# cisco/openh264

Hardware: NVIDIA B200
Metric: 1080p_encode_fps (higher is better)
Workload: dtype u8

## Files before the change

openh264_b200/csrc/enc_batch.cu:

```cuda
#include <atomic>
#include <chrono>
#include <condition_variable>
#include <functional>
#include <mutex>
#include <string.h>
#include <thread>
#include <vector>

#include "../../include/b2h264_codec.h"
#include "b2h264_internal.h"
#include "enc_host.h"
#include "enc_launch.h"
#include "host_pool.h"

using b2h264::StreamCtl;
using b2h264::Pool;
using b2h264::usable_cores;

namespace {

#define CK(x) do { cudaError_t e_ = (x); if (e_ != cudaSuccess) return (int)e_; } while (0)


}

struct b2h264_enc {
  b2h264_enc_config cfg;
  int S = 0, n_mb = 0;
  std::vector<StreamCtl> ctl;
  std::vector<uint8_t> idr_next;
  std::vector<int32_t> p_since_idr;
  std::vector<uint8_t> have_ref_p;
  int cur_rec = 0;
  std::vector<uint8_t> stream_rec;
  cudaStream_t st = nullptr;
  cudaStream_t st_in = nullptr;
  cudaStream_t st_out = nullptr;
  cudaStream_t st_dbk = nullptr;
  uint8_t* d_cur = nullptr;
  int32_t* d_vaa = nullptr;
  uint8_t* d_pic_all = nullptr;
  uint8_t* d_pic[2] = {nullptr, nullptr};
  uint8_t* d_src = nullptr;
  MbInfo* d_mbi = nullptr;
  RefMbInfo* d_rinfo[2] = {nullptr, nullptr};
  MbOut* d_out[2] = {nullptr, nullptr};
  int32_t* d_sad = nullptr;
  int32_t* d_prog = nullptr;
  int32_t* d_bits = nullptr;
  bool mb_bits_on = false;
  int* d_tickets = nullptr;
  void* d_stash = nullptr;
  StreamFrame* d_sf[2] = {nullptr, nullptr};
  alignas(64) unsigned char tmap_pic[128];
  bool have_tmap = false;
  void* d_tmap = nullptr;
  const uint8_t** d_srcptr[2] = {nullptr, nullptr};
  uint8_t* h_src = nullptr;
  MbOut* h_out[2] = {nullptr, nullptr};
  int32_t* h_idx[2] = {nullptr, nullptr};
  int32_t* h_cnt[2] = {nullptr, nullptr};
  unsigned long long last_d2h = 0;
  StreamFrame* h_sf[2] = {nullptr, nullptr};
  const uint8_t** h_srcptr[2] = {nullptr, nullptr};
  struct Slot { bool busy = false; std::vector<uint8_t> idr; std::vector<int> act;
                cudaEvent_t ev0, ev1, ev2, done, in_done, enc_done, ev_ready, ev_dbk; };
  Slot slot[2];
  int submit_idx = 0, collect_idx = 0;
  std::vector<std::vector<uint8_t>> bs;
  Pool* pool = nullptr;
  float last_us[4] = {0, 0, 0, 0};
  bool own_stream = true;
  size_t frame_bytes = 0, cur_bytes = 0, pic_bytes = 0, pic_y_bytes = 0, pic_c_bytes = 0;

  uint8_t* pic_plane0(int set, int s, int pl) const {
    const int sty = ctl[0].rec_stride_y(), stc = ctl[0].rec_stride_c();
    uint8_t* base = d_pic[set] + (size_t)s * pic_bytes;
    if (pl == 0) return base + (size_t)32 * sty + 32;
    return base + pic_y_bytes + (size_t)(pl - 1) * pic_c_bytes + (size_t)16 * stc + 16;
  }
};

extern "C" {

int b2h264_enc_create(const b2h264_enc_config* cfg, b2h264_enc** out) {
  if (!cfg || !out) return -1;
  if (cfg->width < 16 || cfg->height < 16 || (cfg->width & 3) || (cfg->height & 1) || cfg->qp < 0 || cfg->qp > 51 ||
      cfg->n_streams < 1)
    return -2;
  int rc = b2h264_init(cfg->device);
  if (rc) return rc;
  if ((rc = enc_upload_deblock_tables())) return rc;
  b2h264_enc* e = new b2h264_enc();
  e->cfg = *cfg;
  e->S = cfg->n_streams;
  e->ctl.resize(e->S);
  for (auto& c : e->ctl) {
    c.init(cfg->width, cfg->height, cfg->qp, cfg->fps, cfg->target_bitrate, cfg->entropy_cabac, cfg->profile_idc);
    c.fast_mode = cfg->complexity_low != 0;
    if (!c.set_loop_filter(cfg->loop_filter_idc, cfg->loop_filter_alpha_c0_offset, cfg->loop_filter_beta_offset)) { delete e; return -1; }
    c.increasing_ids = cfg->sps_pps_id_strategy != 0;
  }
  e->idr_next.assign(e->S, 1);
  e->p_since_idr.assign(e->S, 0);
  e->have_ref_p.assign(e->S, 0);
  e->stream_rec.assign(e->S, 0);
  const StreamCtl& c0 = e->ctl[0];
  const int mbw = c0.sp.mb_w, mbh = c0.sp.mb_h;
  e->n_mb = mbw * mbh;
  e->frame_bytes = (size_t)cfg->width * cfg->height * 3 / 2;
  e->cur_bytes = (size_t)e->n_mb * 384;
  e->pic_y_bytes = (size_t)c0.rec_stride_y() * c0.rec_rows_y();
  e->pic_c_bytes = (size_t)c0.rec_stride_c() * c0.rec_rows_c();
  e->pic_bytes = (e->pic_y_bytes + 2 * e->pic_c_bytes + 255) & ~(size_t)255;
  const size_t S = e->S;
  CK(cudaStreamCreateWithFlags(&e->st, cudaStreamNonBlocking));
  CK(cudaStreamCreateWithFlags(&e->st_in, cudaStreamNonBlocking));
  CK(cudaStreamCreateWithFlags(&e->st_dbk, cudaStreamNonBlocking));
  {
    int lo = 0, hi = 0;
    cudaDeviceGetStreamPriorityRange(&lo, &hi);
    CK(cudaStreamCreateWithPriority(&e->st_out, cudaStreamNonBlocking, lo));
  }
  CK(cudaMalloc(&e->d_pic_all, 2 * S * e->pic_bytes + 256));
  CK(cudaMemset(e->d_pic_all, 0, 2 * S * e->pic_bytes + 256));
  CK(cudaMalloc(&e->d_cur, 2 * S * e->cur_bytes + 256));
  CK(cudaMemset(e->d_cur, 0, 2 * S * e->cur_bytes + 256));
  CK(cudaMalloc(&e->d_vaa, S * e->n_mb * 4 * sizeof(int32_t)));
  CK(cudaMemset(e->d_vaa, 0, S * e->n_mb * 4 * sizeof(int32_t)));
  for (int i = 0; i < 2; i++) {
    e->d_pic[i] = e->d_pic_all + (size_t)i * S * e->pic_bytes;
    CK(cudaMalloc(&e->d_rinfo[i], S * e->n_mb * sizeof(RefMbInfo)));
    CK(cudaMemset(e->d_rinfo[i], 0, S * e->n_mb * sizeof(RefMbInfo)));
    CK(cudaMalloc(&e->d_out[i], S * e->n_mb * sizeof(MbOut)));
    CK(cudaMalloc(&e->d_sf[i], S * sizeof(StreamFrame)));
    CK(cudaMalloc(&e->d_srcptr[i], S * sizeof(uint8_t*)));
    CK(cudaHostAlloc(&e->h_out[i], S * e->n_mb * sizeof(MbOut), cudaHostAllocMapped));
    CK(cudaHostAlloc(&e->h_idx[i], S * e->n_mb * sizeof(int32_t), cudaHostAllocMapped));
    CK(cudaHostAlloc(&e->h_cnt[i], S * sizeof(int32_t), cudaHostAllocMapped));
    CK(cudaMallocHost(&e->h_sf[i], S * sizeof(StreamFrame)));
    CK(cudaMallocHost(&e->h_srcptr[i], S * sizeof(uint8_t*)));
    CK(cudaEventCreate(&e->slot[i].ev0));
    CK(cudaEventCreate(&e->slot[i].ev1));
    CK(cudaEventCreate(&e->slot[i].ev2));
    CK(cudaEventCreateWithFlags(&e->slot[i].done, cudaEventDisableTiming));
    CK(cudaEventCreateWithFlags(&e->slot[i].in_done, cudaEventDisableTiming));
    CK(cudaEventCreateWithFlags(&e->slot[i].enc_done, cudaEventDisableTiming));
    CK(cudaEventCreateWithFlags(&e->slot[i].ev_ready, cudaEventDisableTiming));
    CK(cudaEventCreateWithFlags(&e->slot[i].ev_dbk, cudaEventDisableTiming));
  }
  e->have_tmap = b2h264_make_tmap_planes(e->tmap_pic, e->d_pic_all, (uint64_t)c0.rec_stride_y(), (uint64_t)c0.rec_rows_y(), 2 * (uint64_t)S,
                                         (uint64_t)c0.rec_stride_y(), (uint64_t)e->pic_bytes, 64, 48) == 0;
  if (e->have_tmap) {
    CK(cudaMalloc(&e->d_tmap, 128));
    CK(cudaMemcpy(e->d_tmap, e->tmap_pic, 128, cudaMemcpyHostToDevice));
  }
  CK(cudaMalloc(&e->d_src, 2 * S * e->frame_bytes + 256));
  CK(cudaMallocHost(&e->h_src, 2 * S * e->frame_bytes));
  CK(cudaMalloc(&e->d_mbi, S * e->n_mb * sizeof(MbInfo)));
  CK(cudaMemset(e->d_mbi, 0, S * e->n_mb * sizeof(MbInfo)));
  CK(cudaMalloc(&e->d_sad, S * e->n_mb * sizeof(int32_t)));
  CK(cudaMemset(e->d_sad, 0, S * e->n_mb * sizeof(int32_t)));
  CK(cudaMalloc(&e->d_prog, S * 2 * mbh * sizeof(int32_t)));
  CK(cudaMalloc(&e->d_bits, S * e->n_mb * sizeof(int32_t)));
  CK(cudaMalloc(&e->d_tickets, enc_sched_ints((int)S, e->n_mb) * sizeof(int)));
  CK(cudaMalloc(&e->d_stash, enc_stash_bytes((int)S, e->ctl[0].sp.mb_h)));
  e->bs.resize(S);
  int nt = cfg->entropy_threads;
  if (nt <= 0) { nt = usable_cores(); if (nt > (int)S) nt = (int)S; if (nt < 1) nt = 1; }
  e->pool = new Pool(nt);
  *out = e;
  return 0;
}

void b2h264_enc_destroy(b2h264_enc* e) {
  if (!e) return;
  cudaSetDevice(e->cfg.device);
  cudaStreamSynchronize(e->st);
  delete e->pool;
  cudaFree(e->d_pic_all); cudaFree(e->d_cur); cudaFree(e->d_vaa); cudaFree(e->d_tmap); cudaFree(e->d_src); cudaFree(e->d_mbi); cudaFree(e->d_sad); cudaFree(e->d_prog); cudaFree(e->d_bits); cudaFree(e->d_tickets); cudaFree(e->d_stash);
  cudaFreeHost(e->h_src);
  for (int i = 0; i < 2; i++) {
    cudaFree(e->d_rinfo[i]); cudaFree(e->d_out[i]); cudaFree(e->d_sf[i]); cudaFree(e->d_srcptr[i]);
    cudaFreeHost(e->h_out[i]); cudaFreeHost(e->h_idx[i]); cudaFreeHost(e->h_cnt[i]); cudaFreeHost(e->h_sf[i]); cudaFreeHost(e->h_srcptr[i]);
    cudaEventDestroy(e->slot[i].ev0); cudaEventDestroy(e->slot[i].ev1); cudaEventDestroy(e->slot[i].ev2); cudaEventDestroy(e->slot[i].done); cudaEventDestroy(e->slot[i].in_done); cudaEventDestroy(e->slot[i].enc_done); cudaEventDestroy(e->slot[i].ev_ready); cudaEventDestroy(e->slot[i].ev_dbk);
  }
  if (e->own_stream) cudaStreamDestroy(e->st);
  cudaStreamDestroy(e->st_in); cudaStreamDestroy(e->st_out); if (e->st_dbk) cudaStreamDestroy(e->st_dbk);
  delete e;
}

int b2h264_enc_force_idr(b2h264_enc* e, int stream) {
  if (!e || stream >= e->S) return -1;
  for (int s = 0; s < e->S; s++) if (stream < 0 || stream == s) e->idr_next[s] = 1;
  return 0;
}

int b2h264_enc_submit(b2h264_enc* e, const uint8_t* const* src, int src_on_device) {
  if (!e || !src) return -1;
  CK(cudaSetDevice(e->cfg.device));
  const int k = e->submit_idx & 1;
  b2h264_enc::Slot& sl = e->slot[k];
  if (sl.busy) return -3;
  const int S = e->S, mbw = e->ctl[0].sp.mb_w, mbh = e->ctl[0].sp.mb_h;
  sl.act.clear();
  for (int s = 0; s < S; s++) if (src[s]) sl.act.push_back(s);
  const int n = (int)sl.act.size();
  if (n == 0) return -5;
  for (int i = 0; i < n; i++) {
    const int s = sl.act[i];
    if (src_on_device) { e->h_srcptr[k][i] = src[s]; continue; }
    uint8_t* dd = e->d_src + ((size_t)k * S + s) * e->frame_bytes;
    e->h_srcptr[k][i] = dd;
    cudaPointerAttributes at;
    const bool pinned = cudaPointerGetAttributes(&at, src[s]) == cudaSuccess && at.type == cudaMemoryTypeHost;
    const uint8_t* from = src[s];
    if (!pinned) {
      (void)cudaGetLastError();
      uint8_t* hs = e->h_src + ((size_t)k * S + s) * e->frame_bytes;
      memcpy(hs, src[s], e->frame_bytes);
      from = hs;
    }
    CK(cudaMemcpyAsync(dd, from, e->frame_bytes, cudaMemcpyHostToDevice, e->st_in));
  }
  sl.idr.assign(S, 0);
  for (int i = 0; i < n; i++) {
    const int s = sl.act[i];
    const bool idr = e->idr_next[s] != 0 || (e->cfg.intra_period > 0 && 1 + e->p_since_idr[s] >= e->cfg.intra_period);
    e->p_since_idr[s] = idr ? 0 : e->p_since_idr[s] + 1;
    sl.idr[s] = idr;
    StreamFrame& F = e->h_sf[k][i];
    F.p = e->ctl[s].frame_params(idr, e->have_ref_p[s] != 0);
    const int cpar = e->stream_rec[s];
    uint8_t* cur = e->d_cur + ((size_t)cpar * S + s) * e->cur_bytes;
    F.f.prev_luma = e->cfg.complexity_low ? e->d_cur + ((size_t)(1 - cpar) * S + s) * e->cur_bytes : nullptr;
    F.f.vaa_sad8x8 = e->cfg.complexity_low ? e->d_vaa + (size_t)s * e->n_mb * 4 : nullptr;
    F.f.cur[0] = cur; F.f.cur[1] = cur + (size_t)e->n_mb * 256; F.f.cur[2] = cur + (size_t)e->n_mb * 320;
    const int prec = e->stream_rec[s];
    F.p.ref_plane = (1 - prec) * S + s;
    for (int pl = 0; pl < 3; pl++) { F.f.rec[pl] = e->pic_plane0(prec, s, pl); F.f.ref[pl] = e->pic_plane0(1 - prec, s, pl); }
    F.f.mbi = e->d_mbi + (size_t)s * e->n_mb;
    F.f.rec_info = e->d_rinfo[prec] + (size_t)s * e->n_mb;
    F.f.ref_info = e->d_rinfo[1 - prec] + (size_t)s * e->n_mb;
    F.f.out = e->d_out[k] + (size_t)i * e->n_mb;
    F.f.sad_cost = e->d_sad + (size_t)s * e->n_mb;
    F.f.mb_bits = e->mb_bits_on ? e->d_bits + (size_t)s * e->n_mb : nullptr;
    e->idr_next[s] = 0;
    e->have_ref_p[s] = !idr;
  }
  for (int i = 0; i < n; i++) e->stream_rec[sl.act[i]] ^= 1;
  if (!src_on_device) {
    CK(cudaEventRecord(sl.in_done, e->st_in));
    CK(cudaStreamWaitEvent(e->st, sl.in_done, 0));
  }
  CK(cudaMemcpyAsync(e->d_sf[k], e->h_sf[k], n * sizeof(StreamFrame), cudaMemcpyHostToDevice, e->st));
  CK(cudaMemcpyAsync(e->d_srcptr[k], e->h_srcptr[k], n * sizeof(uint8_t*), cudaMemcpyHostToDevice, e->st));
  CK(cudaEventRecord(sl.ev0, e->st));
  int rc = enc_launch_frame(e->d_sf[k], e->d_srcptr[k], n, e->cfg.width, e->cfg.height, mbw, mbh, e->d_tickets, e->d_stash,
                            e->have_tmap ? e->tmap_pic : nullptr, e->d_tmap, e->cfg.complexity_low != 0, e->st, e->st_dbk, sl.ev_ready, sl.ev_dbk);
  if (rc) return rc;
  CK(cudaEventRecord(sl.ev1, e->st));
  rc = enc_launch_deblock_expand(e->d_sf[k], n, mbw, mbh, e->d_tickets, e->st, sl.ev_dbk);
  if (rc) return rc;
  CK(cudaEventRecord(sl.ev2, e->st));
  CK(cudaStreamWaitEvent(e->st_out, sl.ev1, 0));
  rc = enc_launch_pack(e->d_sf[k], n, e->n_mb, e->h_out[k], e->h_idx[k], e->h_cnt[k], e->st_out);
  if (rc) return rc;
  CK(cudaEventRecord(sl.done, e->st_out));
  sl.busy = true;
  e->submit_idx++;
  return 0;
}

int b2h264_enc_collect(b2h264_enc* e, const uint8_t** bs, int32_t* bs_bytes, int32_t* frame_type) {
  if (!e) return -1;
  CK(cudaSetDevice(e->cfg.device));
  const int k = e->collect_idx & 1;
  b2h264_enc::Slot& sl = e->slot[k];
  if (!sl.busy) return -4;
  CK(cudaEventSynchronize(sl.done));
  float ms = 0;
  cudaEventElapsedTime(&ms, sl.ev0, sl.ev1);
  e->last_us[0] = ms * 1000.f;
  if (cudaEventQuery(sl.ev2) == cudaSuccess && cudaEventElapsedTime(&ms, sl.ev1, sl.ev2) == cudaSuccess)
    e->last_us[1] = ms * 1000.f;
  (void)cudaGetLastError();
  const auto t0 = std::chrono::steady_clock::now();
  const int n_mb = e->n_mb, n = (int)sl.act.size();
  e->last_d2h = (unsigned long long)n * (n_mb + 1) * sizeof(int32_t);
  for (int i = 0; i < n; i++) e->last_d2h += (unsigned long long)e->h_cnt[k][i] * 32;
  for (int s = 0; s < e->S; s++) e->bs[s].clear();
  std::function<void(int)> job = [&](int i) {
    const int s = sl.act[i];
    e->ctl[s].write_access_unit_packed(sl.idr[s] != 0, e->h_out[k] + (size_t)i * n_mb, e->h_idx[k] + (size_t)i * n_mb, &e->bs[s]);
  };
  e->pool->run(n, job);
  e->last_us[2] = std::chrono::duration<float, std::micro>(std::chrono::steady_clock::now() - t0).count();
  std::vector<uint8_t> active(e->S, 0);
  for (int i = 0; i < n; i++) active[sl.act[i]] = 1;
  for (int s = 0; s < e->S; s++) {
    if (bs) bs[s] = active[s] ? e->bs[s].data() : nullptr;
    if (bs_bytes) bs_bytes[s] = (int32_t)e->bs[s].size();
    if (frame_type) frame_type[s] = !active[s] ? 0 : sl.idr[s] ? 1 : 2;
  }
  sl.busy = false;
  e->collect_idx++;
  return 0;
}

int b2h264_enc_reset_stream(b2h264_enc* e, int stream) {
  if (!e || stream < 0 || stream >= e->S) return -1;
  if (e->slot[0].busy || e->slot[1].busy) return -3;
  CK(cudaSetDevice(e->cfg.device));
  e->ctl[stream] = StreamCtl();
  e->ctl[stream].init(e->cfg.width, e->cfg.height, e->cfg.qp, e->cfg.fps, e->cfg.target_bitrate, e->cfg.entropy_cabac, e->cfg.profile_idc);
  e->ctl[stream].increasing_ids = e->cfg.sps_pps_id_strategy != 0;
  e->ctl[stream].fast_mode = e->cfg.complexity_low != 0;
  e->ctl[stream].set_loop_filter(e->cfg.loop_filter_idc, e->cfg.loop_filter_alpha_c0_offset, e->cfg.loop_filter_beta_offset);
  e->ctl[stream].record_mb_bits = e->mb_bits_on;
  e->idr_next[stream] = 1;
  e->p_since_idr[stream] = 0;
  e->have_ref_p[stream] = 0;
  CK(cudaMemsetAsync(e->d_sad + (size_t)stream * e->n_mb, 0, e->n_mb * sizeof(int32_t), e->st));
  for (int i = 0; i < 2; i++) CK(cudaMemsetAsync(e->d_rinfo[i] + (size_t)stream * e->n_mb, 0, e->n_mb * sizeof(RefMbInfo), e->st));
  CK(cudaMemsetAsync(e->d_mbi + (size_t)stream * e->n_mb, 0, e->n_mb * sizeof(MbInfo), e->st));
  CK(cudaStreamSynchronize(e->st));
  return 0;
}

int b2h264_enc_set_mb_bits(b2h264_enc* e, int on) {
  if (!e) return -1;
  if (e->slot[0].busy || e->slot[1].busy) return -3;
  e->mb_bits_on = on != 0;
  for (auto& c : e->ctl) c.record_mb_bits = on != 0;
  return 0;
}

int b2h264_enc_get_mb_bits(b2h264_enc* e, int stream, int32_t* device_bits, int32_t* host_bits) {
  if (!e || stream < 0 || stream >= e->S || !e->mb_bits_on) return -1;
  if (e->slot[0].busy || e->slot[1].busy) return -3;
  CK(cudaSetDevice(e->cfg.device));
  CK(cudaStreamSynchronize(e->st));
  if (device_bits) CK(cudaMemcpy(device_bits, e->d_bits + (size_t)stream * e->n_mb, e->n_mb * sizeof(int32_t), cudaMemcpyDeviceToHost));
  if (host_bits) {
    if ((int)e->ctl[stream].last_mb_bits.size() != e->n_mb) return -1;
    memcpy(host_bits, e->ctl[stream].last_mb_bits.data(), e->n_mb * sizeof(int32_t));
  }
  return 0;
}

int b2h264_enc_last_coded_mbs(b2h264_enc* e, unsigned long long* count) {
  if (!e || !count) return -1;
  unsigned long long n = 0;
  for (const auto& c : e->ctl) n += (unsigned long long)c.last_coded_mbs;
  *count = n;
  return 0;
}
int b2h264_enc_last_d2h_bytes(b2h264_enc* e, unsigned long long* bytes) {
  if (!e || !bytes) return -1;
  *bytes = e->last_d2h;
  return 0;
}

int b2h264_enc_get_recon(b2h264_enc* e, int stream, uint8_t* dst) {
  if (!e || stream < 0 || stream >= e->S || !dst) return -1;
  CK(cudaSetDevice(e->cfg.device));
  CK(cudaStreamSynchronize(e->st));
  const int set = 1 - e->stream_rec[stream];
  const int w = e->cfg.width, h = e->cfg.height;
  for (int pl = 0; pl < 3; pl++) {
    const int pw = pl ? w / 2 : w, ph = pl ? h / 2 : h;
    const int st = pl ? e->ctl[0].rec_stride_c() : e->ctl[0].rec_stride_y();
    CK(cudaMemcpy2D(dst, pw, e->pic_plane0(set, stream, pl), st, pw, ph, cudaMemcpyDeviceToHost));
    dst += (size_t)pw * ph;
  }
  return 0;
}

int b2h264_enc_last_timing(b2h264_enc* e, float* us3) {
  if (!e || !us3) return -1;
  us3[0] = e->last_us[0]; us3[1] = e->last_us[1]; us3[2] = e->last_us[2];
  return 0;
}

int b2h264_enc_set_stream(b2h264_enc* e, void* stream) {
  if (!e) return -1;
  if (e->slot[0].busy || e->slot[1].busy) return -3;
  CK(cudaStreamSynchronize(e->st));
  if (e->own_stream) cudaStreamDestroy(e->st);
  e->st = (cudaStream_t)stream;
  e->own_stream = false;
  return 0;
}

}
```

openh264_b200/csrc/enc_frame.cuh:

```cuda
#pragma once
#include "enc_mb.cuh"
#include "enc_cavlc_bits.cuh"
#ifdef B2H264_WITH_INTER
#include "enc_inter.cuh"
#endif

namespace mbk {

MBK_HD void mb_ctx(MbCtx& c, const EncFrameParams& p, const EncFramePtrs& f, int mbx, int mby) {
  static_assert(sizeof(EncFrameParams) % 4 == 0 && sizeof(EncFramePtrs) % 4 == 0, "copied as words");
  warp_sync();
  const uint32_t* sp = reinterpret_cast<const uint32_t*>(&p);
  const uint32_t* sfp = reinterpret_cast<const uint32_t*>(&f);
  uint32_t* dp = reinterpret_cast<uint32_t*>(&c.p);
  uint32_t* df = reinterpret_cast<uint32_t*>(&c.f);
  for (int i = lane_id(); i < (int)(sizeof(EncFrameParams) / 4); i += MBK_WS) dp[i] = sp[i];
  for (int i = lane_id(); i < (int)(sizeof(EncFramePtrs) / 4); i += MBK_WS) df[i] = sfp[i];
  if (lane_id() == 0) {
    c.mbx = mbx; c.mby = mby;
    c.nb = (mbx > 0 ? NB_LEFT : 0) | (mby > 0 ? NB_TOP : 0) | (mbx > 0 && mby > 0 ? NB_TOPLEFT : 0) |
           (mby > 0 && mbx < p.mb_w - 1 ? NB_TOPRIGHT : 0);
    c.qp = p.qp;
    c.qp_c = tbl_chroma_qp(p.qp);
    c.lambda = tbl_lambda(p.qp);
    c.tmap_ref = nullptr; c.wbar = nullptr; c.win_mode = 0;
  }
  warp_sync();
}

#ifndef B2H264_WITH_INTER
enum { MBS_DONE = 0, MBS_A = 1, MBS_I = 2, MBS_BSKIP = 3, MBS_B = 4, MBS_C = 5, MBS_COUNT = 6 };
#endif

MBK_HD int mb_run_stage(const MbCtx& c, MbScratch& s, int stage) {
  int next = MBS_DONE;
  if (stage == MBS_A || stage == MBS_I) {
    phase_mark(s, 31);
    uint32_t* a = reinterpret_cast<uint32_t*>(&s.info);
    for (int i = lane_id(); i < (int)(sizeof(MbInfo) / 4); i += MBK_WS) a[i] = 0;
    uint32_t* b = reinterpret_cast<uint32_t*>(&s.out);
    for (int i = lane_id(); i < MBOUT_HEADER_WORDS; i += MBK_WS) b[i] = 0;
    mb_load_all(c, s);
    phase_mark(s, 0);
  } else {
    mb_load_cur(c, s);
  }
  if (stage == MBS_I) {
    intra_mb_md_enc(c, s, 0x7fffffff);
    if (lane_id() == 0) { s.info.ref_idx = -1; c.f.sad_cost[c.mby * c.p.mb_w + c.mbx] = 0; }
  }
#ifdef B2H264_WITH_INTER
  else if (stage == MBS_A) next = inter_stage_a(c, s);
  else if (stage == MBS_B || stage == MBS_BSKIP) next = inter_stage_b(c, s);
  else if (stage == MBS_C) next = inter_stage_c(c, s);
#endif
  warp_sync();
  if (next == MBS_DONE) {
    phase_mark(s, 10);
    if (s.info.mb_type == MBT_PSKIP && s.st.is_skip != 0) mb_store_recon_skip(c, s);
    else mb_store_recon(c, s);
    mb_publish(c, s);
    if (c.f.mb_bits != nullptr) {
      const int b = mb_cavlc_bits(c, s);
      if (lane_id() == 0) c.f.mb_bits[c.mby * c.p.mb_w + c.mbx] = b;
    }
    phase_mark(s, 11);
  }
  return next;
}

MBK_HD void encode_one_mb(const EncFrameParams& p, const EncFramePtrs& f, MbScratch& s, int mbx, int mby) {
  mb_ctx(s.ctx, p, f, mbx, mby);
  int stage = p.is_idr ? MBS_I : MBS_A;
  while (stage != MBS_DONE) stage = mb_run_stage(s.ctx, s, stage);
}

}
```

openh264_b200/csrc/enc_inter.cuh:

```cuda
#pragma once
#include "enc_mb.cuh"
#include "mbk_mc.cuh"
#include "mbk_me.cuh"

namespace mbk {

#define REF_NOT_AVAIL (-2)
#define REF_NOT_IN_LIST (-1)

MBK_HD int cache30(int k) { return 7 + blk_y(k) * 6 + blk_x(k); }


MBK_HD int median3(int a, int b, int c) {
  const int mn = a < b ? a : b, mx = a < b ? b : a;
  return c < mn ? mn : (c > mx ? mx : c);
}

MBK_HD int nb_slot_bit(int k) {
  return (int)((((uint32_t)NB_TOPLEFT) | ((uint32_t)NB_TOP << 8) | ((uint32_t)NB_TOPRIGHT << 16) | ((uint32_t)NB_LEFT << 24)) >> (8 * k)) & 0xff;
}
MBK_FN void fill_inter_cache(const MbCtx& c, MbScratch& s, bool ref_ids = false) {
  for (int ci = lane_id(); ci < 30; ci += MBK_WS) {
    int k = -1, blk = 0;
    if (ci == 0) { k = 0; blk = 15; }
    else if (ci <= 4) { k = 1; blk = 12 + ci - 1; }
    else if (ci == 5) { k = 2; blk = 12; }
    else if (ci % 6 == 0) { k = 3; blk = 4 * (ci / 6 - 1) + 3; }
    int16_t mx = 0, my = 0;
    int8_t ref = 0;
    if (k >= 0) {
      const bool avail = (c.nb & nb_slot_bit(k)) != 0;
      const MbInfo* n = &s.nbi[k];
      if (avail && MBT_IS_INTER(n->mb_type)) { mx = n->mv[blk][0]; my = n->mv[blk][1]; if (ref_ids) ref = n->i4_mode[blk]; }
      else ref = avail ? REF_NOT_IN_LIST : REF_NOT_AVAIL;
    } else if (ci == 9 || ci == 11 || ci == 17 || ci == 21 || ci == 23) {
      ref = REF_NOT_AVAIL;
    }
    s.mvc[ci][0] = mx; s.mvc[ci][1] = my; s.refc[ci] = ref;
  }
  for (int k = lane_id(); k < 4; k += MBK_WS) {
    const bool avail = (c.nb & nb_slot_bit(k)) != 0;
    const MbInfo* n = &s.nbi[k];
    const bool inter = avail && MBT_IS_INTER(n->mb_type);
    const bool skip = inter && n->mb_type == MBT_PSKIP;
    s.sadc[k] = inter ? s.nb_sad[k] : 0;
    s.skip_flag[k] = skip;
    s.sad_skip[k] = skip ? s.nb_skip_sad[k] : 0;
  }
  warp_sync();
}

MBK_FN void pred_mv(const MbScratch& s, int blk , int part_w, int ref, int* px, int* py) {
  const int left = cache30(blk) - 1, top = cache30(blk) - 6;
  const int lr = s.refc[left], tr = s.refc[top], rtr = s.refc[top + part_w];
  int dr, dmx, dmy;
  if (rtr == REF_NOT_AVAIL) { dr = s.refc[top - 1]; dmx = s.mvc[top - 1][0]; dmy = s.mvc[top - 1][1]; }
  else { dr = rtr; dmx = s.mvc[top + part_w][0]; dmy = s.mvc[top + part_w][1]; }
  if (tr == REF_NOT_AVAIL && dr == REF_NOT_AVAIL && lr != REF_NOT_AVAIL) { *px = s.mvc[left][0]; *py = s.mvc[left][1]; return; }
  const int match = (ref == lr ? 1 : 0) | (ref == tr ? 2 : 0) | (ref == dr ? 4 : 0);
  if (match == 1) { *px = s.mvc[left][0]; *py = s.mvc[left][1]; }
  else if (match == 2) { *px = s.mvc[top][0]; *py = s.mvc[top][1]; }
  else if (match == 4) { *px = dmx; *py = dmy; }
  else { *px = median3(s.mvc[left][0], s.mvc[top][0], dmx); *py = median3(s.mvc[left][1], s.mvc[top][1], dmy); }
}
MBK_HD void pred_16x8_mv(const MbScratch& s, int blk, int ref, int* px, int* py) {
  if (blk == 0) { if (ref == s.refc[1]) { *px = s.mvc[1][0]; *py = s.mvc[1][1]; return; } }
  else { if (ref == s.refc[18]) { *px = s.mvc[18][0]; *py = s.mvc[18][1]; return; } }
  pred_mv(s, blk, 4, ref, px, py);
}
MBK_HD void pred_8x16_mv(const MbScratch& s, int blk, int ref, int* px, int* py) {
  if (blk == 0) { if (ref == s.refc[6]) { *px = s.mvc[6][0]; *py = s.mvc[6][1]; return; } }
  else {
    int di = 5;
    if (s.refc[5] == REF_NOT_AVAIL) di = 2;
    if (ref == s.refc[di]) { *px = s.mvc[di][0]; *py = s.mvc[di][1]; return; }
  }
  pred_mv(s, blk, 2, ref, px, py);
}
MBK_HD void pred_skip_mv(const MbScratch& s, int* px, int* py, int ref0 = 0 ) {
  const int lr = s.refc[6], tr = s.refc[1];
  if (lr == REF_NOT_AVAIL || tr == REF_NOT_AVAIL || (lr == ref0 && s.mvc[6][0] == 0 && s.mvc[6][1] == 0) ||
      (tr == ref0 && s.mvc[1][0] == 0 && s.mvc[1][1] == 0)) { *px = 0; *py = 0; return; }
  pred_mv(s, 0, 4, ref0, px, py);
}
MBK_HD void cache_set(MbScratch& s, int blk, int w4, int h4, int mvx, int mvy, int ref = 0) {
  if (lane_id() == 0) {
    const int c0 = cache30(blk);
    for (int y = 0; y < h4; y++)
      for (int x = 0; x < w4; x++) { s.mvc[c0 + 6 * y + x][0] = (int16_t)mvx; s.mvc[c0 + 6 * y + x][1] = (int16_t)mvy; s.refc[c0 + 6 * y + x] = (int8_t)ref; }
  }
  warp_sync();
}
MBK_HD void mb_mv_set(MbScratch& s, int blk, int w4, int h4, int mvx, int mvy) {
  if (lane_id() == 0) {
    const int x0 = blk_x(blk), y0 = blk_y(blk);
    for (int y = 0; y < h4; y++)
      for (int x = 0; x < w4; x++) { s.info.mv[(y0 + y) * 4 + x0 + x][0] = (int16_t)mvx; s.info.mv[(y0 + y) * 4 + x0 + x][1] = (int16_t)mvy; }
  }
  warp_sync();
}

MBK_HD int predict_sad(const MbScratch& s) {
  const int rb = s.refc[1], ra = s.refc[6];
  int rc = s.refc[5], sc = s.sadc[2];
  const int sb = s.sadc[1], sa = s.sadc[3];
  if (rc == REF_NOT_AVAIL) { rc = s.refc[0]; sc = s.sadc[0]; }
  int pred;
  if (rb == REF_NOT_AVAIL && rc == REF_NOT_AVAIL && ra != REF_NOT_AVAIL) pred = sa;
  else {
    const int m = (0 == ra ? 1 : 0) | (0 == rb ? 2 : 0) | (0 == rc ? 4 : 0);
    pred = m == 1 ? sa : m == 2 ? sb : m == 4 ? sc : median3(sa, sb, sc);
  }
  const int t = pred << 6;
  return ((t - (t >> 3) + (t >> 5)) + 32) >> 6;
}
MBK_HD int predict_sad_skip(const MbScratch& s) {
  const int rb = s.refc[1], ra = s.refc[6];
  int rc = s.refc[5];
  const int sb = s.skip_flag[1] ? s.sad_skip[1] : 0, sa = s.skip_flag[3] ? s.sad_skip[3] : 0;
  int sc = s.skip_flag[2] ? s.sad_skip[2] : 0, rskip = s.skip_flag[2];
  if (rc == REF_NOT_AVAIL) { rc = s.refc[0]; sc = s.skip_flag[0] ? s.sad_skip[0] : 0; rskip = s.skip_flag[0]; }
  if (rb == REF_NOT_AVAIL && rc == REF_NOT_AVAIL && ra != REF_NOT_AVAIL) return sa;
  const int m = ((0 == ra && s.skip_flag[3]) ? 1 : 0) | ((0 == rb && s.skip_flag[1]) ? 2 : 0) | ((0 == rc && rskip) ? 4 : 0);
  return m == 1 ? sa : m == 2 ? sb : m == 4 ? sc : median3(sa, sb, sc);
}

MBK_HD const uint8_t* ref_luma(const MbCtx& c, int px, int py) {
  return c.f.ref[0] + (ptrdiff_t)(c.mby * 16 + py) * c.p.rec_stride_y + c.mbx * 16 + px;
}
MBK_HD const uint8_t* ref_chroma(const MbCtx& c, int pl, int px, int py) {
  return c.f.ref[pl] + (ptrdiff_t)(c.mby * 8 + py) * c.p.rec_stride_c + c.mbx * 8 + px;
}

MBK_STAGE void mc_chroma_part(const MbCtx& c, uint8_t* dst , int ox, int oy, int w, int h, int mvx, int mvy) {
  const int cx = ox >> 1, cy = oy >> 1;
  MBK_NO_UNROLL
  for (int pl = 0; pl < 2; pl++) {
    const uint8_t* src = ref_chroma(c, 1 + pl, cx + (mvx >> 3), cy + (mvy >> 3));
    warp_mc_chroma(src, c.p.rec_stride_c, dst + 64 * pl + cy * 8 + cx, 8, mvx, mvy, w >> 1, h >> 1);
  }
  warp_sync();
}

struct SkipResult { bool ok; int cost_luma; int cost_skip; int mvx, mvy; };

MBK_STAGE bool try_py_skip(const MbCtx& c, MbScratch& s) {
  const int16_t* ff = tbl_quant_ff(c.qp);
  const int16_t* mf = tbl_quant_mf(c.qp);
  int big = 0, ctr = 0;
  for (int k = lane_id(); k < 16; k += MBK_WS) {
    int16_t d[16], l[16];
    for (int i = 0; i < 16; i++) d[i] = s.coef[16 * k + i];
    const uint16_t mx = (uint16_t)quant4x4_max(d, ff, mf);
    if (mx > 1) big = 1;
    else if (mx == 1) { scan4x4_dcac(l, d); ctr += single_ctr4x4(l); }
  }
  big = warp_sum(big); ctr = warp_sum(ctr);
  return big == 0 && ctr < 6;
}
MBK_STAGE bool try_puv_skip(const MbCtx& c, MbScratch& s, int uv) {
  const int16_t* res = s.coef + 256 + 64 * uv;
  const int16_t* ff = tbl_quant_ff(c.qp_c);
  const int16_t* mf = tbl_quant_mf(c.qp_c);
  const int16_t dcin[4] = {res[0], res[16], res[32], res[48]};
  const bool dc_fail = hadamard_quant2x2_skip(dcin, (int16_t)(ff[0] << 1), (int16_t)(mf[0] >> 1)) != 0;
  int big = 0, ctr = 0;
  for (int j = lane_id(); j < 4; j += MBK_WS) {
    int16_t d[16], l[16];
    for (int i = 0; i < 16; i++) d[i] = res[16 * j + i];
    const uint16_t mx = (uint16_t)quant4x4_max(d, ff, mf);
    if (mx > 1) big = 1;
    else if (mx == 1) { scan4x4_ac(l, d); ctr += single_ctr4x4(l); }
  }
  big = warp_sum(big); ctr = warp_sum(ctr);
  return !dc_fail && big == 0 && ctr < 7;
}
MBK_FN void dct_luma_mb(MbScratch& s, const uint8_t* pred ) {
  for (int k = lane_id(); k < 16; k += MBK_WS) {
    int16_t d[16];
    const int o = blk_y(k) * 4 * 16 + blk_x(k) * 4;
    dct4x4(d, s.cur_y + o, 16, pred + o, 16);
    for (int i = 0; i < 16; i++) s.coef[16 * k + i] = d[i];
  }
  warp_sync();
}

MBK_STAGE SkipResult pskip_enc(const MbCtx& c, MbScratch& s, int sad_pred_skip, int ref_mb_type) {
  SkipResult r;
  r.ok = false; r.cost_luma = 0; r.cost_skip = 0;
  int mvx, mvy;
  pred_skip_mv(s, &mvx, &mvy);
  r.mvx = mvx; r.mvy = mvy;
  const int ix = mvx >> 2, iy = mvy >> 2;
  int n = c.mbx * 16 + ix;
  if (n < -29 || n > c.p.mb_w * 16 + 12) return r;
  n = c.mby * 16 + iy;
  if (n < -29 || n > c.p.mb_h * 16 + 12) return r;
  uint8_t* py = s.skip_pred;
  phase_mark(s, 12);
  warp_mc_luma(ref_luma(c, ix, iy), c.p.rec_stride_y, py, 16, mvx, mvy, 16, 16);
  warp_sync();
  phase_mark(s, 13);
  const int sad_y = warp_sad(s.cur_y, 16, py, 16, 4, 4);
  MBK_NO_UNROLL
  for (int pl = 0; pl < 2; pl++)
    warp_mc_chroma(ref_chroma(c, 1 + pl, ix >> 1, iy >> 1), c.p.rec_stride_c, s.skip_pred + 256 + 64 * pl, 8, mvx, mvy, 8, 8);
  warp_sync();
  const int sad_c = warp_sad(s.cur_c, 8, s.skip_pred + 256, 8, 3, 3) + warp_sad(s.cur_c + 64, 8, s.skip_pred + 320, 8, 3, 3);
  const int sad_mb = sad_y + sad_c;
  phase_mark(s, 14);
  bool ok = sad_mb == 0 || sad_mb < sad_pred_skip ||
            (c.p.ref_is_p && ref_mb_type == MBT_PSKIP && sad_mb < c.f.ref_info[c.mby * c.p.mb_w + c.mbx].skip_sad);
  if (!ok) {
    dct_luma_mb(s, py);
    if (try_py_skip(c, s)) {
      for (int t = lane_id(); t < 4; t += MBK_WS) {
        int16_t d[16];
        const int ox = (t & 1) * 4, oy = (t >> 1) * 4;
        dct4x4(d, s.cur_c + oy * 8 + ox, 8, s.skip_pred + 256 + oy * 8 + ox, 8);
        for (int i = 0; i < 16; i++) s.coef[256 + 16 * t + i] = d[i];
      }
      warp_sync();
      bool uv_ok = true;
      MBK_NO_UNROLL
      for (int uv = 0; uv < 2 && uv_ok; uv++) {
        if (uv) {
          for (int t = lane_id(); t < 4; t += MBK_WS) {
            int16_t d[16];
            const int ox = (t & 1) * 4, oy = (t >> 1) * 4;
            dct4x4(d, s.cur_c + 64 + oy * 8 + ox, 8, s.skip_pred + 320 + oy * 8 + ox, 8);
            for (int i = 0; i < 16; i++) s.coef[320 + 16 * t + i] = d[i];
          }
          warp_sync();
        }
        uv_ok = try_puv_skip(c, s, uv);
      }
      ok = uv_ok;
    }
  }
  phase_mark(s, 15);
  if (ok) {
    r.ok = true;
    if (c.p.fast_mode) {
      r.cost_luma = sad_y;
      if (lane_id() == 0) c.f.sad_cost[c.mby * c.p.mb_w + c.mbx] = sad_y;
    } else {
      r.cost_luma = warp_satd_inl(s.cur_y, 16, py, 16, 4, 4);
    }
    phase_mark(s, 16);
    r.cost_skip = sad_mb;
  }
  return r;
}

MBK_HD void win_issue(const MbCtx& c, MbScratch& s, int sx, int sy) {
#ifdef __CUDA_ARCH__
  warp_sync();
  if (c.win_mode == 0) { if (lane_id() == 0) s.win_ok = 0; warp_sync(); return; }
  const int X = (32 + c.mbx * 16 + sx - 16) & ~15, Y = 32 + c.mby * 16 + sy - 16, Z = c.p.ref_plane;
  const int wx0 = X - 32 - c.mbx * 16;
  if (lane_id() == 0) { s.win_x0 = wx0; s.win_y0 = sy - 16; s.win_ok = 1; }
  if (c.win_mode == 1) {
    if (lane_id() == 0) {
      const uint32_t dst = (uint32_t)__cvta_generic_to_shared(scratch_win(s));
      const uint32_t bar = (uint32_t)__cvta_generic_to_shared(&c.wbar->bar);
      asm volatile("fence.proxy.async.shared::cta;" ::: "memory");
      asm volatile("{ .reg .b64 st; mbarrier.arrive.expect_tx.shared::cta.b64 st, [%0], %1; }" ::"r"(bar), "r"(WIN_W * WIN_H) : "memory");
      asm volatile("cp.async.bulk.tensor.3d.shared::cluster.global.mbarrier::complete_tx::bytes [%0], [%1, {%2, %3, %4}], [%5];"
                   ::"r"(dst), "l"(c.tmap_ref), "r"(X), "r"(Y), "r"(Z), "r"(bar) : "memory");
    }
  } else {
    const uint32_t* src = reinterpret_cast<const uint32_t*>(ref_luma(c, wx0, sy - 16));
    uint32_t* dst = reinterpret_cast<uint32_t*>(scratch_win(s));
    const int rs4 = c.p.rec_stride_y >> 2;
#pragma unroll 8
    for (int i = lane_id(); i < WIN_H * (WIN_W / 4); i += MBK_WS) {
      const int r = i / (WIN_W / 4), w = i - r * (WIN_W / 4);
      dst[i] = src[(ptrdiff_t)r * rs4 + w];
    }
  }
  warp_sync();
#else
  (void)c; (void)sx; (void)sy;
  s.win_ok = 0;
#endif
}
MBK_HD void win_wait(const MbCtx& c, MbScratch& s) {
#ifdef __CUDA_ARCH__
  if (c.win_mode == 1 && s.win_ok) {
    const uint32_t bar = (uint32_t)__cvta_generic_to_shared(&c.wbar->bar);
    const uint32_t ph = c.wbar->phase;
    uint32_t ok = 0;
    while (!ok)
      asm volatile("{ .reg .pred p; mbarrier.try_wait.parity.shared::cta.b64 p, [%1], %2; selp.u32 %0, 1, 0, p; }"
                   : "=r"(ok) : "r"(bar), "r"(ph) : "memory");
    warp_sync();
    if (lane_id() == 0) c.wbar->phase = ph ^ 1;
    warp_sync();
  }
#else
  (void)c; (void)s;
#endif
}

MBK_STAGE void me_partition(const MbCtx& c, MbScratch& s, int blk_size, int ox, int oy, int mvp_x, int mvp_y, uint32_t sad_pred,
                         int n_mvc, const int16_t* mvc, MeState* st) {
  MeIn in;
  in.enc = s.cur_y + oy * 16 + ox; in.enc_stride = 16;
  in.ref = ref_luma(c, ox, oy); in.ref_stride = c.p.rec_stride_y;
  in.blk = blk_size;
  in.mvp_x = mvp_x; in.mvp_y = mvp_y;
  const int r = c.p.mv_range;
  const int lo_x = -((c.mbx + 1) << 4) + 3, lo_y = -((c.mby + 1) << 4) + 3;
  const int hi_x = ((c.p.mb_w - c.mbx) << 4) - 3, hi_y = ((c.p.mb_h - c.mby) << 4) - 3;
  in.min_x = lo_x > -r ? lo_x : -r; in.min_y = lo_y > -r ? lo_y : -r;
  in.max_x = hi_x < r ? hi_x : r; in.max_y = hi_y < r ? hi_y : r;
  in.n_mvc = n_mvc; in.mvc = mvc;
  in.sad_pred = sad_pred;
  in.lambda = c.lambda;
  in.calc_satd = !c.p.fast_mode;
  in.win = s.win_ok ? scratch_win(s) : nullptr;
  in.win_w = WIN_W; in.win_h = WIN_H;
  in.win_dx = s.win_x0 - ox; in.win_dy = s.win_y0 - oy;
  MeOut o;
  warp_me_search(in, o);
  if (lane_id() == 0) {
    st->mv_x = o.mv_x; st->mv_y = o.mv_y; st->mvp_x = mvp_x; st->mvp_y = mvp_y;
    st->sad_cost = o.sad_cost; st->satd_cost = o.satd_cost;
    st->satd = (int)o.satd_cost - mvd_cost(c.lambda, o.mv_x - mvp_x, o.mv_y - mvp_y);
    st->ref = o.ref_best;
  }
  warp_sync();
}
MBK_HD void me_start_point(const MbCtx& c, int mvp_x, int mvp_y, int* sx, int* sy) {
  const int r = c.p.mv_range;
  const int lo_x = -((c.mbx + 1) << 4) + 3, lo_y = -((c.mby + 1) << 4) + 3;
  const int hi_x = ((c.p.mb_w - c.mbx) << 4) - 3, hi_y = ((c.p.mb_h - c.mby) << 4) - 3;
  *sx = clip3((2 + mvp_x) >> 2, lo_x > -r ? lo_x : -r, hi_x < r ? hi_x : r);
  *sy = clip3((2 + mvp_y) >> 2, lo_y > -r ? lo_y : -r, hi_y < r ? hi_y : r);
}

struct QpelPlanes { const uint8_t* g; const uint8_t* hh; const uint8_t* vv; const uint8_t* cc; };
enum { QP_STRIDE = 32 };
MBK_HD void qpel_pair(const QpelPlanes& q, int dx, int dy, const uint8_t** pa, const uint8_t** pb) {
  const int ix = dx < 0 ? -1 : 0, iy = dy < 0 ? -1 : 0, fx = dx & 3, fy = dy & 3;
  const uint8_t* G = q.g + (iy + 3) * QP_STRIDE + (ix + 3);
  const uint8_t* H = q.hh + (iy + 1) * QP_STRIDE + (ix + 1);
  const uint8_t* V = q.vv + (iy + 1) * QP_STRIDE + (ix + 1);
  const uint8_t* C = q.cc + (iy + 1) * QP_STRIDE + (ix + 1);
  const int x3 = fx == 3 ? 1 : 0, y3 = fy == 3 ? QP_STRIDE : 0;
  if ((fx | fy) == 0) { *pa = G; *pb = G; }
  else if (fy == 0) { *pa = H; *pb = fx == 2 ? H : G + x3; }
  else if (fx == 0) { *pa = V; *pb = fy == 2 ? V : G + y3; }
  else if (fx == 2 && fy == 2) { *pa = C; *pb = C; }
  else if (fx == 2) { *pa = H + y3; *pb = C; }
  else if (fy == 2) { *pa = V + x3; *pb = C; }
  else { *pa = H + y3; *pb = V + x3; }
}

MBK_STAGE void me_refine(const MbCtx& c, MbScratch& s, MeState* st, int ox, int oy, int w, int h, uint8_t* dst) {
  const int lw = w == 16 ? 4 : 3, lh = h == 16 ? 4 : 3;
  const uint8_t* enc = s.cur_y + oy * 16 + ox;
  const int rs = c.p.rec_stride_y;
  const int px = st->mvp_x, py = st->mvp_y;
  const int mv0x = st->mv_x, mv0y = st->mv_y;
  const uint8_t* ref0 = st->ref;
  int best = (c.p.fast_mode ? warp_satd(enc, 16, ref0, rs, lw, lh) : st->satd) + mvd_cost(c.lambda, mv0x - px, mv0y - py);
  uint8_t* win = reinterpret_cast<uint8_t*>(s.coef);
  static_assert(sizeof(s.coef) >= 22 * QP_STRIDE, "window aliases the coefficient buffer");
  const int ww = w + 6, wh = h + 6, wq = (ww + 3) >> 2;
  const uint8_t* src = ref0 - (ptrdiff_t)3 * rs - 3;
  int srs = rs;
  if (s.win_ok) {
    const int x0 = ox + (mv0x >> 2) - 3 - s.win_x0, y0 = oy + (mv0y >> 2) - 3 - s.win_y0;
    if (x0 >= 0 && y0 >= 0 && x0 + 4 * wq <= WIN_W && y0 + wh <= WIN_H) { src = scratch_win(s) + y0 * WIN_W + x0; srs = WIN_W; }
  }
#ifdef __CUDA_ARCH__
  {
    uint32_t v[5];
#pragma unroll
    for (int k = 0; k < 5; k++) {
      const int i = lane_id() + 32 * k;
      const int r = i / wq, q4 = (i - r * wq) << 2;
      v[k] = i < wq * wh ? ld4u(src + (ptrdiff_t)r * srs + q4) : 0u;
    }
    warp_sync();
#pragma unroll
    for (int k = 0; k < 5; k++) {
      const int i = lane_id() + 32 * k;
      if (i < wq * wh) {
        const int r = i / wq, q4 = (i - r * wq) << 2;
        uint8_t* d = win + r * QP_STRIDE + q4;
        d[0] = (uint8_t)v[k]; d[1] = (uint8_t)(v[k] >> 8); d[2] = (uint8_t)(v[k] >> 16); d[3] = (uint8_t)(v[k] >> 24);
      }
    }
  }
#else
  for (int i = lane_id(); i < wq * wh; i += MBK_WS) {
    const int r = i / wq, q4 = (i - r * wq) << 2;
    const uint32_t v = ld4u(src + (ptrdiff_t)r * srs + q4);
    uint8_t* d = win + r * QP_STRIDE + q4;
    d[0] = (uint8_t)v; d[1] = (uint8_t)(v >> 8); d[2] = (uint8_t)(v >> 16); d[3] = (uint8_t)(v >> 24);
  }
#endif
  warp_sync();
  if (lane_id() == 0) s.win_ok = 0;
  warp_sync();
  uint8_t* ph = s.qplane[0];
  uint8_t* pv = s.qplane[1];
  uint8_t* pc = s.qplane[2];
  for (int i = lane_id(); i < (w + 1) * (h + 2); i += MBK_WS) {
    const int r = i / (w + 1), x = i - r * (w + 1);
    ph[r * QP_STRIDE + x] = (uint8_t)half_h(win + (r + 2) * QP_STRIDE + (x + 2));
  }
  for (int i = lane_id(); i < (w + 2) * (h + 1); i += MBK_WS) {
    const int r = i / (w + 2), x = i - r * (w + 2);
    pv[r * QP_STRIDE + x] = (uint8_t)half_v(win + (r + 2) * QP_STRIDE + (x + 2), QP_STRIDE);
  }
  warp_sync();
  QpelPlanes q;
  q.g = win; q.hh = ph; q.vv = pv; q.cc = pc;
  auto eval = [&](int dx, int dy) {
    const uint8_t *a, *b;
    qpel_pair(q, dx, dy, &a, &b);
    return warp_satd_avg(enc, 16, a, b, QP_STRIDE, lw, lh) + mvd_cost(c.lambda, mv0x + dx - px, mv0y + dy - py);
  };
  int hx = 0, hy = 0;
  {
    int bi = -1;
    MBK_NO_UNROLL
    for (int i = 0; i < 4; i++) {
      const int cst = eval(i == 2 ? -2 : i == 3 ? 2 : 0, i == 0 ? -2 : i == 1 ? 2 : 0);
      if (cst < best) { best = cst; bi = i; }
    }
    if (bi >= 0) { hx = bi == 2 ? -2 : bi == 3 ? 2 : 0; hy = bi == 0 ? -2 : bi == 1 ? 2 : 0; }
  }
  if (hx | hy) {
    for (int i = lane_id(); i < (w + 1) * (h + 1); i += MBK_WS) {
      const int r = i / (w + 1), x = i - r * (w + 1);
      pc[r * QP_STRIDE + x] = (uint8_t)half_c(win + (r + 2) * QP_STRIDE + (x + 2), QP_STRIDE);
    }
    warp_sync();
  }
  int fx = hx, fy = hy;
  {
    int bi = -1;
    MBK_NO_UNROLL
    for (int i = 0; i < 4; i++) {
      const int cst = eval(hx + (i == 2 ? -1 : i == 3 ? 1 : 0), hy + (i == 0 ? -1 : i == 1 ? 1 : 0));
      if (cst < best) { best = cst; bi = i; }
    }
    if (bi >= 0) { fx += (bi == 2 ? -1 : bi == 3 ? 1 : 0); fy += (bi == 0 ? -1 : bi == 1 ? 1 : 0); }
  }
  {
    const uint8_t *a, *b;
    qpel_pair(q, fx, fy, &a, &b);
    const int gsh = lw - 2;
    for (int g = lane_id(); g < (w * h) >> 2; g += MBK_WS) {
      const int y = g >> gsh, x = (g & ((1 << gsh) - 1)) << 2;
      const uint32_t v = vavgu4(ld4u(a + y * QP_STRIDE + x), ld4u(b + y * QP_STRIDE + x));
      uint8_t* d = dst + y * 16 + x;
      d[0] = (uint8_t)v; d[1] = (uint8_t)(v >> 8); d[2] = (uint8_t)(v >> 16); d[3] = (uint8_t)(v >> 24);
    }
    warp_sync();
  }
  if (lane_id() == 0) { st->mv_x = mv0x + fx; st->mv_y = mv0y + fy; st->satd_cost = (uint32_t)best; }
  warp_sync();
}

MBK_STAGE void enc_inter_y(const MbCtx& c, MbScratch& s) {
  const int16_t* ff = tbl_quant_ff(c.qp);
  const int16_t* mf = tbl_quant_mf(c.qp);
  for (int k = lane_id(); k < 16; k += MBK_WS) {
    int16_t d[16], l[16];
    for (int i = 0; i < 16; i++) d[i] = s.coef[16 * k + i];
    const int16_t mx = quant4x4_max(d, ff, mf);
    if (mx == 0) { for (int i = 0; i < 16; i++) l[i] = 0; }
    else scan4x4_dcac(l, d);
    for (int i = 0; i < 16; i++) { s.coef[16 * k + i] = d[i]; s.out.luma[k][i] = l[i]; }
    s.red[k] = mx;
    s.red[16 + k] = mx == 0 ? 0 : single_ctr4x4(l);
  }
  warp_sync();
  int ctr8[4], ctr_mb = 0;
  for (int i = 0; i < 4; i++) {
    ctr8[i] = 0;
    for (int j = 0; j < 4; j++) {
      const int mx = s.red[4 * i + j];
      if (mx == 0) continue;
      if (mx > 1) ctr8[i] += 9;
      else if (ctr8[i] < 6) ctr8[i] += s.red[16 + 4 * i + j];
    }
    ctr_mb += ctr8[i];
  }
  for (int i = lane_id(); i < 16; i += MBK_WS) s.info.nnz[i] = 0;
  warp_sync();
  if (ctr_mb < 6) {
    for (int i = lane_id(); i < 256; i += MBK_WS) s.coef[i] = 0;
  } else {
    for (int k = lane_id(); k < 16; k += MBK_WS) {
      if (ctr8[k >> 2] >= 4) {
        s.info.nnz[blk_raster(k)] = (int8_t)nonzero_count(s.out.luma[k]);
        int16_t d[16];
        for (int i = 0; i < 16; i++) d[i] = s.coef[16 * k + i];
        dequant4x4(d, tbl_dequant(c.qp));
        for (int i = 0; i < 16; i++) s.coef[16 * k + i] = d[i];
      } else {
        for (int i = 0; i < 16; i++) s.coef[16 * k + i] = 0;
      }
    }
    if (lane_id() == 0)
      for (int i = 0; i < 4; i++) if (ctr8[i] >= 4) s.info.cbp |= (uint8_t)(1 << i);
  }
  warp_sync();
}

MBK_FN void rec_luma_inter(MbScratch& s, const uint8_t* pred) {
  for (int k = lane_id(); k < 16; k += MBK_WS) {
    int16_t d[16];
    for (int i = 0; i < 16; i++) d[i] = s.coef[16 * k + i];
    const int oy = blk_y(k) * 4, ox = blk_x(k) * 4;
    idct4x4_rec(tile_y(s.tile, ox, oy), TY_PITCH, pred + oy * 16 + ox, 16, d);
  }
  warp_sync();
}

MBK_HD void decided_pskip(const MbCtx& c, MbScratch& s) {
  (void)c;
  if (lane_id() == 0) {
    s.info.mb_type = MBT_PSKIP;
    s.info.cbp = 0;
  }
  for (int i = lane_id(); i < 24; i += MBK_WS) s.info.nnz[i] = 0;
  warp_sync();
}

enum { MBS_DONE = 0, MBS_A = 1, MBS_I = 2, MBS_BSKIP = 3, MBS_B = 4, MBS_C = 5, MBS_COUNT = 6 };

MBK_FN void inter_tail(const MbCtx& c, MbScratch& s) {
  const int idx = c.mby * c.p.mb_w + c.mbx;
  const int final_type = s.st.final_type, p16_mvx = s.st.p16_mvx, p16_mvy = s.st.p16_mvy, cost_skip_mb = s.st.cost_skip_mb;
  if (lane_id() == 0) {
    s.info.mb_type = (uint8_t)final_type;
    s.info.p16x16_mv[0] = (int16_t)p16_mvx; s.info.p16x16_mv[1] = (int16_t)p16_mvy;
    if (MBT_IS_INTER(final_type)) s.info.ref_idx = 0;
    RefMbInfo ri;
    ri.mv16[0] = (int16_t)p16_mvx; ri.mv16[1] = (int16_t)p16_mvy;
    ri.skip_sad = final_type == MBT_PSKIP ? cost_skip_mb : 0;
    ri.mb_type = (uint8_t)final_type;
    ri.pad[0] = ri.pad[1] = ri.pad[2] = 0;
    c.f.rec_info[idx] = ri;
  }
  warp_sync();
}

MBK_HD void st_save(MbScratch& s, int is_skip, int cost_luma, int cost_skip_mb, int p16_mvx, int p16_mvy, int final_type) {
  warp_sync();
  if (lane_id() == 0) {
    s.st.is_skip = is_skip; s.st.cost_luma = cost_luma; s.st.cost_skip_mb = cost_skip_mb;
    s.st.p16_mvx = p16_mvx; s.st.p16_mvy = p16_mvy; s.st.final_type = final_type;
  }
  warp_sync();
}

MBK_STAGE int inter_stage_a(const MbCtx& c, MbScratch& s) {
  const int mbw = c.p.mb_w, idx = c.mby * mbw + c.mbx;
  fill_inter_cache(c, s);
  mbk_batch_sync(5, c.batch_n);
  phase_mark(s, 1);
  const int ref_mb_type = c.p.ref_is_p ? c.f.ref_info[idx].mb_type : 0xff;
  int p16_mvx = 0, p16_mvy = 0;
  const bool sk_l = (c.nb & NB_LEFT) && s.nbi[3].mb_type == MBT_PSKIP;
  const bool sk_t = (c.nb & NB_TOP) && s.nbi[1].mb_type == MBT_PSKIP;
  const bool sk_tl = (c.nb & NB_TOPLEFT) && s.nbi[0].mb_type == MBT_PSKIP;
  const bool sk_tr = (c.nb & NB_TOPRIGHT) && s.nbi[2].mb_type == MBT_PSKIP;
  const bool try_skip = sk_l || sk_t || sk_tl || sk_tr;
  const bool keep_skip = sk_l && sk_t && sk_tr;
  int cost_luma = 0, cost_skip_mb = 0;
  bool is_skip = false;
  if ((c.p.ref_is_p && ref_mb_type == MBT_PSKIP) || try_skip) {
    const SkipResult r = pskip_enc(c, s, predict_sad_skip(s), ref_mb_type);
    if (r.ok) {
      is_skip = true;
      cost_luma = r.cost_luma; cost_skip_mb = r.cost_skip;
      p16_mvx = r.mvx; p16_mvy = r.mvy;
      mb_mv_set(s, 0, 4, 4, r.mvx, r.mvy);
    }
  }
  mbk_batch_sync(6, c.batch_n);
  phase_mark(s, 2);
  if (is_skip && keep_skip) {
    decided_pskip(c, s);
    st_save(s, 1, cost_luma, cost_skip_mb, p16_mvx, p16_mvy, MBT_PSKIP);
    inter_tail(c, s);
    return MBS_DONE;
  }
  st_save(s, is_skip ? 1 : 0, cost_luma, cost_skip_mb, p16_mvx, p16_mvy, MBT_P16x16);
  return is_skip ? MBS_BSKIP : MBS_B;
}

MBK_STAGE int inter_stage_b(const MbCtx& c, MbScratch& s) {
  const int mbw = c.p.mb_w, idx = c.mby * mbw + c.mbx;
  const bool is_skip = s.st.is_skip != 0;
  int cost_luma = s.st.cost_luma, cost_skip_mb = s.st.cost_skip_mb, p16_mvx = s.st.p16_mvx, p16_mvy = s.st.p16_mvy;
  MeState& me16 = s.me[0];
  MeState* me16x8 = &s.me[1];
  MeState* me8x16 = &s.me[3];
  MeState* me8x8 = &s.me[5];
  int final_type = MBT_P16x16;
  int sad_pred_mb = 0;
  if (lane_id() == 0) s.win_ok = 0;
  warp_sync();
  int16_t (*mvc)[2] = s.mvcand;
  int px16 = 0, py16 = 0, n16 = 1;
  if (!is_skip) {
    pred_mv(s, 0, 4, 0, &px16, &py16);
    {
      int sx, sy;
      me_start_point(c, px16, py16, &sx, &sy);
      win_issue(c, s, sx, sy);
    }
    sad_pred_mb = predict_sad(s);
    n16 += (c.nb & NB_LEFT) ? 1 : 0;
    n16 += (c.nb & NB_TOP) ? 1 : 0;
    if (c.p.ref_is_p) { n16 += c.mbx < mbw - 1 ? 1 : 0; n16 += c.mby < c.p.mb_h - 1 ? 1 : 0; }
    if (lane_id() == 0) {
      int k = 0;
      mvc[k][0] = 0; mvc[k][1] = 0; k++;
      if (c.nb & NB_LEFT) { mvc[k][0] = s.nbi[3].p16x16_mv[0]; mvc[k][1] = s.nbi[3].p16x16_mv[1]; k++; }
      if (c.nb & NB_TOP) { mvc[k][0] = s.nbi[1].p16x16_mv[0]; mvc[k][1] = s.nbi[1].p16x16_mv[1]; k++; }
      if (c.p.ref_is_p) {
        if (c.mbx < mbw - 1) { mvc[k][0] = c.f.ref_info[idx + 1].mv16[0]; mvc[k][1] = c.f.ref_info[idx + 1].mv16[1]; k++; }
        if (c.mby < c.p.mb_h - 1) { mvc[k][0] = c.f.ref_info[idx + mbw].mv16[0]; mvc[k][1] = c.f.ref_info[idx + mbw].mv16[1]; k++; }
      }
    }
    warp_sync();
    win_wait(c, s);
  }
  int plan[3] = {0, 0, 0}, n_plan = 0, cost = 0;
  int rounds_run = 0;
  MBK_NO_UNROLL
  for (int t = -1; t < n_plan; t++) {
    const int shape = t < 0 ? 0 : plan[t];
    int cst = 0;
    if (t >= 0 || !is_skip) {
      const int np = shape == 0 ? 1 : shape == 3 ? 4 : 2;
      MeState* arr = shape == 0 ? &me16 : shape == 1 ? me16x8 : shape == 2 ? me8x16 : me8x8;
      MBK_NO_UNROLL
      for (int i = 0; i < np; i++) {
        int px = px16, py = py16, ox = 0, oy = 0, blk = BLK_16x16, ci = 0, cw = 4, ch = 4, ncand = n16;
        uint32_t sp = (uint32_t)sad_pred_mb;
        if (shape == 1) { pred_16x8_mv(s, 8 * i, 0, &px, &py); oy = 8 * i; blk = BLK_16x8; ci = 8 * i; ch = 2; sp = (uint32_t)(sad_pred_mb >> 1); ncand = 1; }
        else if (shape == 2) { pred_8x16_mv(s, 4 * i, 0, &px, &py); ox = 8 * i; blk = BLK_8x16; ci = 4 * i; cw = 2; sp = (uint32_t)(sad_pred_mb >> 1); ncand = 1; }
        else if (shape == 3) { pred_mv(s, 4 * i, 2, 0, &px, &py); ox = (i & 1) * 8; oy = (i >> 1) * 8; blk = BLK_8x8; ci = 4 * i; cw = 2; ch = 2; sp = (uint32_t)(sad_pred_mb >> 2); ncand = 1; }
        me_partition(c, s, blk, ox, oy, px, py, sp, ncand, &mvc[0][0], &arr[i]);
        if (shape != 0) cache_set(s, ci, cw, ch, arr[i].mv_x, arr[i].mv_y);
        cst += (int)arr[i].satd_cost;
      }
    }
    if (t >= 0) {
      mbk_batch_sync(7 + t, c.batch_n_fine);
      rounds_run = t + 1;
      if (t == 0) { if (cst < cost_luma) { cost = cst; final_type = shape == 3 ? MBT_P8x8 : shape == 1 ? MBT_P16x8 : MBT_P8x16; } else break; }
      else if (cst <= cost) { cost = cst; final_type = shape == 1 ? MBT_P16x8 : MBT_P8x16; }
      continue;
    }
    if (!is_skip) { p16_mvx = me16.mv_x; p16_mvy = me16.mv_y; cost_luma = cst; }
    if (!is_skip) mbk_batch_sync(2, c.batch_n);
    phase_mark(s, 3);
    {
      int bb;
      const int cost16 = md_i16x16_inl(c, s, &bb);
      phase_mark(s, 4);
      if (cost16 < cost_luma) {
        st_save(s, is_skip ? 1 : 0, cost_luma, cost_skip_mb, p16_mvx, p16_mvy, final_type);
        if (lane_id() == 0) { s.st.cost16 = cost16; s.st.bb = bb; }
        warp_sync();
        if (!is_skip) {
          mbk_batch_leave(3, c.batch_n); mbk_batch_leave(4, c.batch_n);
          for (int r = 0; r < 3; r++) mbk_batch_leave(7 + r, c.batch_n_fine);
        }
        return MBS_C;
      }
    }
    if (is_skip) {
      decided_pskip(c, s);
      st_save(s, 1, cost_luma, cost_skip_mb, p16_mvx, p16_mvy, MBT_PSKIP);
      inter_tail(c, s);
      return MBS_DONE;
    }
    int vaa_sign = 0;
    if (c.p.fast_mode) {
      const int32_t* v = c.f.vaa_sad8x8 + 4 * idx;
      const int b0 = v[0], b1 = v[1], b2 = v[2], b3 = v[3], avg = (b0 + b1 + b2 + b3) >> 2;
      const int d0 = (b0 >> 6) - (avg >> 6), d1 = (b1 >> 6) - (avg >> 6), d2 = (b2 >> 6) - (avg >> 6), d3 = (b3 >> 6) - (avg >> 6);
      if (d0 * d0 + d1 * d1 + d2 * d2 + d3 * d3 < 20) vaa_sign = 15;
      else vaa_sign = (b0 > avg ? 8 : 0) | (b1 > avg ? 4 : 0) | (b2 > avg ? 2 : 0) | (b3 > avg ? 1 : 0);
    }
    if (c.p.fast_mode && vaa_sign == 15) n_plan = 0;
    else if (c.p.fast_mode && (vaa_sign == 3 || vaa_sign == 12)) { plan[0] = 1; n_plan = 1; }
    else if (c.p.fast_mode && (vaa_sign == 5 || vaa_sign == 10)) { plan[0] = 2; n_plan = 1; }
    else if (c.p.fast_mode && (vaa_sign == 6 || vaa_sign == 9)) { plan[0] = 3; n_plan = 1; }
    else { plan[0] = 3; plan[1] = 1; plan[2] = 2; n_plan = 3; }
  }
  {
    for (int r = rounds_run; r < 3; r++) mbk_batch_leave(7 + r, c.batch_n_fine);
    mbk_batch_sync(3, c.batch_n);
    phase_mark(s, 6);
    uint8_t* pl = s.pred_y[0];
    uint8_t* pc = s.pred_c[0];
    int best_sad = 0;
    {
      const int shape = final_type == MBT_P16x16 ? 0 : final_type == MBT_P16x8 ? 1 : final_type == MBT_P8x16 ? 2 : 3;
      const int np = shape == 0 ? 1 : shape == 3 ? 4 : 2;
      MeState* arr = shape == 0 ? &me16 : shape == 1 ? me16x8 : shape == 2 ? me8x16 : me8x8;
      if (shape == 3) {
        if (lane_id() == 0) { s.refc[9] = s.refc[21] = REF_NOT_AVAIL; }
        warp_sync();
      }
      MBK_NO_UNROLL
      for (int i = 0; i < np; i++) {
        int ox = 0, oy = 0, w = 16, h = 16, ci = 0, cw = 4, ch = 4;
        if (shape != 0) {
          int qx, qy;
          if (shape == 1) { pred_16x8_mv(s, 8 * i, 0, &qx, &qy); oy = 8 * i; h = 8; ci = 8 * i; ch = 2; }
          else if (shape == 2) { pred_8x16_mv(s, 4 * i, 0, &qx, &qy); ox = 8 * i; w = 8; ci = 4 * i; cw = 2; }
          else { pred_mv(s, 4 * i, 2, 0, &qx, &qy); ox = (i & 1) * 8; oy = (i >> 1) * 8; w = 8; h = 8; ci = 4 * i; cw = 2; ch = 2; }
          if (lane_id() == 0) { arr[i].mvp_x = qx; arr[i].mvp_y = qy; }
          warp_sync();
        }
        me_refine(c, s, &arr[i], ox, oy, w, h, pl + oy * 16 + ox);
        cache_set(s, ci, cw, ch, arr[i].mv_x, arr[i].mv_y);
        mb_mv_set(s, ci, cw, ch, arr[i].mv_x, arr[i].mv_y);
        if (lane_id() == 0) { s.out.mvd[i][0] = (int16_t)(arr[i].mv_x - arr[i].mvp_x); s.out.mvd[i][1] = (int16_t)(arr[i].mv_y - arr[i].mvp_y); }
        best_sad += (int)arr[i].sad_cost;
        mc_chroma_part(c, pc, ox, oy, w, h, arr[i].mv_x, arr[i].mv_y);
      }
      if (shape == 0)
        cost_skip_mb = warp_sad(s.cur_y, 16, pl, 16, 4, 4) + warp_sad(s.cur_c, 8, pc, 8, 3, 3) + warp_sad(s.cur_c + 64, 8, pc + 64, 8, 3, 3);
    }
    if (lane_id() == 0) c.f.sad_cost[idx] = best_sad;
    mbk_batch_sync(4, c.batch_n);
    phase_mark(s, 7);
    if (lane_id() == 0) s.info.cbp = 0;
    warp_sync();
    dct_luma_mb(s, pl);
    enc_inter_y(c, s);
    dct_chroma(s, pc);
    enc_rec_uv(c, s, 0, true);
    enc_rec_uv(c, s, 1, true);
    rec_luma_inter(s, pl);
    rec_chroma(s, pc);
    if (final_type == MBT_P16x16 && s.info.cbp == 0) {
      int sx, sy;
      pred_skip_mv(s, &sx, &sy);
      if (sx == me16.mv_x && sy == me16.mv_y) final_type = MBT_PSKIP;
    }
    if (lane_id() == 0) s.info.mb_type = (uint8_t)final_type;
    warp_sync();
  }
  phase_mark(s, 8);
  st_save(s, 0, cost_luma, cost_skip_mb, p16_mvx, p16_mvy, final_type);
  inter_tail(c, s);
  return MBS_DONE;
}

MBK_STAGE int inter_stage_c(const MbCtx& c, MbScratch& s) {
  const int idx = c.mby * c.p.mb_w + c.mbx;
  const int bb = s.st.bb;
  int cost = s.st.cost16;
  {
    {
      bool use_i4 = false;
      if (lane_id() == 0) { s.info.mb_type = MBT_I16x16; s.info.cbp = 0; }
      warp_sync();
      fill_i4_cache(c, s);
      if (intra_try_i4x4(c, s)) {
        const int cost4 = md_enc_i4x4(c, s, cost);
        if (cost4 < cost) { use_i4 = true; cost = cost4; if (lane_id() == 0) s.info.mb_type = MBT_I4x4; warp_sync(); }
      }
      if (!use_i4) {
    if (lane_id() == 0) s.info.cbp = 0;
    warp_sync();
    enc_rec_i16x16(c, s, s.pred_y[bb]);
  }
      int cb;
      md_chroma(c, s, &cb);
      dct_chroma(s, s.pred_c[cb]);
      enc_rec_uv(c, s, 0, false);
      enc_rec_uv(c, s, 1, false);
      rec_chroma(s, s.pred_c[cb]);
      if (lane_id() == 0) { c.f.sad_cost[idx] = 0; s.info.ref_idx = REF_NOT_IN_LIST; }
      phase_mark(s, 5);
    }
  }
  warp_sync();
  if (lane_id() == 0) s.st.final_type = s.info.mb_type;
  warp_sync();
  inter_tail(c, s);
  return MBS_DONE;
}

MBK_FN void inter_mb_md_enc(const MbCtx& c, MbScratch& s) {
  int nx = inter_stage_a(c, s);
  if (nx == MBS_B || nx == MBS_BSKIP) nx = inter_stage_b(c, s);
  if (nx == MBS_C) inter_stage_c(c, s);
}

}
```

openh264_b200/csrc/enc_kernels.cu:

```cuda
#include <cuda.h>
#include <type_traits>
#include <stddef.h>
#include <stdlib.h>
#include <string.h>

#include "b2h264_internal.h"
#define B2H264_WITH_INTER 1
#include "enc_deblock.cuh"
#include "enc_frame.cuh"
#include "dec_mb.cuh"
#include "enc_launch.h"

using namespace mbk;

namespace mbk {
__constant__ uint8_t c_alpha[52];
__constant__ uint8_t c_beta[52];
__constant__ uint8_t c_tc0[52][3];
}

#define DEC_WPC 24
#ifndef ENC_WPC
#define ENC_WPC 23
#endif

__device__ __forceinline__ int ld_volatile(const int* p) { return *reinterpret_cast<const volatile int*>(p); }

__global__ void k_pad_source(const StreamFrame* __restrict__ sf, const uint8_t* const* __restrict__ src, int w, int h) {
  const StreamFrame& F = sf[blockIdx.z];
  const uint8_t* yuv = src[blockIdx.z];
  const int W = F.p.mb_w * 16, H = F.p.mb_h * 16;
  const int x = (blockIdx.x * blockDim.x + threadIdx.x) * 4, y = blockIdx.y * blockDim.y + threadIdx.y;
  if (x >= W || y >= H) return;
  uchar4 v = make_uchar4(0, 0, 0, 0);
  if (y < h) {
    const uint8_t* r = yuv + (size_t)y * w;
    if (x + 3 < w) v = *reinterpret_cast<const uchar4*>(r + x);
  }
  *reinterpret_cast<uchar4*>(const_cast<uint8_t*>(F.f.cur[0]) + (size_t)y * F.p.cur_stride_y + x) = v;
  if (y < H / 2 && x < W / 2) {
    const int cw = w / 2, ch = h / 2;
    for (int pl = 0; pl < 2; pl++) {
      uchar4 c = make_uchar4(0x80, 0x80, 0x80, 0x80);
      const uint8_t* p = yuv + (size_t)w * h + (size_t)pl * cw * ch + (size_t)y * cw;
      if (y < ch) {
        uint8_t t[4];
        for (int i = 0; i < 4; i++) t[i] = (x + i < cw) ? p[x + i] : 0x80;
        c = make_uchar4(t[0], t[1], t[2], t[3]);
      }
      *reinterpret_cast<uchar4*>(const_cast<uint8_t*>(F.f.cur[1 + pl]) + (size_t)y * F.p.cur_stride_c + x) = c;
    }
  }
}

__global__ void __launch_bounds__(256) k_vaa_sad8x8(const StreamFrame* __restrict__ sf, int n_mb) {
  const int lane = threadIdx.x & 31, mb = blockIdx.x * (blockDim.x >> 5) + (threadIdx.x >> 5);
  if (mb >= n_mb) return;
  const StreamFrame& F = sf[blockIdx.y];
  if (F.f.vaa_sad8x8 == nullptr || F.f.prev_luma == nullptr) return;
  const int st = F.p.cur_stride_y, mbx = mb % F.p.mb_w, mby = mb / F.p.mb_w;
  const size_t off = (size_t)(mby * 16 + (lane >> 1)) * st + mbx * 16 + (lane & 1) * 8;
  const uint2 a = *reinterpret_cast<const uint2*>(F.f.cur[0] + off), b = *reinterpret_cast<const uint2*>(F.f.prev_luma + off);
  int v = (int)(__vsadu4(a.x, b.x) + __vsadu4(a.y, b.y));
  v += __shfl_xor_sync(0xffffffffu, v, 2);
  v += __shfl_xor_sync(0xffffffffu, v, 4);
  v += __shfl_xor_sync(0xffffffffu, v, 8);
  if ((lane & 14) == 0) const_cast<int32_t*>(F.f.vaa_sad8x8)[(size_t)mb * 4 + (lane >> 4) * 2 + (lane & 1)] = v;
}

struct Sched {
  int* dep;
  int* queue;
  int* head;
  int* tail;
};

__device__ __forceinline__ void sched_push(const Sched& q, int id) {
  const int slot = atomicAdd(q.tail, 1);
  *reinterpret_cast<volatile int*>(q.queue + slot) = id;
}
__device__ __forceinline__ void sched_notify(const Sched& q, int id, int need) {
  if (atomicAdd(q.dep + id, 1) + 1 == need) sched_push(q, id);
}

template <class Body>
__device__ __forceinline__ void run_mbs(const StreamFrame* sf, int n_streams, const Sched q, Body body) {
  const int lane = threadIdx.x & 31;
  const int mb_w = sf[0].p.mb_w, mb_h = sf[0].p.mb_h, n_mb = mb_w * mb_h, total = n_streams * n_mb;
  for (;;) {
    int id = 0;
    if (lane == 0) {
      const int t = atomicAdd(q.head, 1);
      id = -1;
      if (t < total) {
        while ((id = ld_volatile(q.queue + t)) < 0) __nanosleep(100);
      }
    }
    id = __shfl_sync(MBK_FULL, id, 0);
    if (id < 0) break;
    __threadfence();
    const int si = id / n_mb, mb = id - si * n_mb, y = mb / mb_w, x = mb - y * mb_w;
    body(sf[si], x, y);
    __threadfence();
    __syncwarp();
    if (lane == 0) {
      if (x + 1 < mb_w) sched_notify(q, id + 1, 1 + (y > 0));
      if (y + 1 < mb_h) {
        if (x > 0) sched_notify(q, id + mb_w - 1, 1 + (x - 1 > 0));
        if (x == mb_w - 1) sched_notify(q, id + mb_w, 1 + (x > 0));
      }
    }
  }
}

enum { NQ = MBS_COUNT - 1 };
struct EncSched {
  int* dep;
  int* queue;
  int* ctl;
  uint4* stash;
  int* rowprog;
};
__device__ __forceinline__ int* ctl_head(const EncSched& q, int k) { return q.ctl + 32 * k; }
__device__ __forceinline__ int* ctl_tail(const EncSched& q, int k) { return q.ctl + 32 * k + 1; }
__device__ __forceinline__ int* ctl_done(const EncSched& q) { return q.ctl + 32 * NQ; }
constexpr int kCtlInts = 32 * (NQ + 1);
constexpr int kStashU4 = kParkSlot / 16, kCoreU4 = kParkCore / 16;
static_assert(kParkSlot % 16 == 0 && kParkCore % 16 == 0, "parked ranges are copied as uint4");
__device__ __forceinline__ void park_extra(int stage, int* off, int* n) {
  if (stage == MBS_BSKIP) { *off = (int)(offsetof(MbScratch, skip_pred) / 16); *n = 384 / 16; }
  else if (stage == MBS_C) { *off = (int)(offsetof(MbScratch, pred_y) / 16); *n = 512 / 16; }
  else { *off = 0; *n = 0; }
}

__device__ __forceinline__ void esched_push(const EncSched& q, int total, int stage, int id) {
  const int k = stage - 1;
  const int slot = atomicAdd(ctl_tail(q, k), 1);
  *reinterpret_cast<volatile int*>(q.queue + (size_t)k * total + slot) = id;
}

__device__ unsigned long long g_batch_stats[NQ + 1][3];
__device__ unsigned long long g_task_wall[NQ][2];
__device__ unsigned long long g_fill_stats[NQ][ENC_WPC + 1][2];
extern "C" int b2h264_debug_task_wall(unsigned long long* out, int reset) {
  cudaError_t e = cudaMemcpyFromSymbol(out, g_task_wall, sizeof(g_task_wall));
  if (e == cudaSuccess && reset) { unsigned long long z[NQ][2] = {}; e = cudaMemcpyToSymbol(g_task_wall, z, sizeof(z)); }
  return (int)e;
}
extern "C" int b2h264_debug_fill_stats(unsigned long long* out, int* n_lists, int* wpc, int reset) {
  *n_lists = NQ; *wpc = ENC_WPC;
  cudaError_t e = cudaMemcpyFromSymbol(out, g_fill_stats, sizeof(g_fill_stats));
  if (reset) { void* a = nullptr; if (cudaGetSymbolAddress(&a, g_fill_stats) == cudaSuccess) cudaMemset(a, 0, sizeof(g_fill_stats)); }
  return (int)e;
}
extern "C" int b2h264_debug_batch_stats(unsigned long long* out, int reset) {
  cudaError_t e = cudaMemcpyFromSymbol(out, g_batch_stats, sizeof(g_batch_stats));
  if (e == cudaSuccess && reset) { unsigned long long z[NQ + 1][3] = {}; e = cudaMemcpyToSymbol(g_batch_stats, z, sizeof(z)); }
  return (int)e;
}

template <class Body>
__device__ __forceinline__ void run_task(const StreamFrame* sf, const EncSched& q, MbScratch& s, int id, int stage, int mb_w, int mb_h,
                                         int total, int batch_n, Body& body) {
  const int lane = threadIdx.x & 31, n_mb = mb_w * mb_h;
  __threadfence();
  const int si = id / n_mb, mb = id - si * n_mb, y = mb / mb_w, x = mb - y * mb_w;
  uint4* park = q.stash + (size_t)(si * mb_h + y) * kStashU4;
  uint4* sc = reinterpret_cast<uint4*>(&s);
  if (stage != MBS_A && stage != MBS_I) {
    int xo, xn;
    park_extra(stage, &xo, &xn);
    for (int i = lane; i < kCoreU4 + xn; i += 32) {
      const uint4 v = __ldcg(park + i);
      if (i < kCoreU4) sc[i] = v; else sc[xo + i - kCoreU4] = v;
    }
    __syncwarp();
  }
  const int next = body(sf[si], x, y, stage, batch_n);
  __syncwarp();
  if (next == MBS_DONE) {
    __threadfence();
    if (lane == 0) {
      const int first = sf[si].p.is_idr ? MBS_I : MBS_A;
      const bool nr = x + 1 < mb_w;
      const bool nbl = y + 1 < mb_h && x > 0;
      const bool nb = y + 1 < mb_h && x == mb_w - 1;
      const int r0 = nr ? atomicAdd(q.dep + id + 1, 1) : 0;
      const int r1 = nbl ? atomicAdd(q.dep + id + mb_w - 1, 1) : 0;
      const int r2 = nb ? atomicAdd(q.dep + id + mb_w, 1) : 0;
      if (nr && r0 + 1 == 1 + (y > 0)) esched_push(q, total, first, id + 1);
      if (nbl && r1 + 1 == 1 + (x - 1 > 0)) esched_push(q, total, first, id + mb_w - 1);
      if (nb && r2 + 1 == 1 + (x > 0)) esched_push(q, total, first, id + mb_w);
      if (q.rowprog) atomicAdd(q.rowprog + si * mb_h + y, 1);
      atomicAdd(ctl_done(q), 1);
    }
  } else {
    int xo, xn;
    park_extra(next, &xo, &xn);
    for (int i = lane; i < kCoreU4 + xn; i += 32) park[i] = i < kCoreU4 ? sc[i] : sc[xo + i - kCoreU4];
    __threadfence();
    __syncwarp();
    if (lane == 0) esched_push(q, total, next, id);
  }
}

struct BatchSlot { int k, base, n, pad; };
constexpr int kEncThreads = 32 * (ENC_WPC + 1);
__device__ __forceinline__ void enc_cta_barrier() { asm volatile("barrier.sync 1, %0;" ::"n"(kEncThreads) : "memory"); }

template <class Body>
__device__ __forceinline__ void run_stages(const StreamFrame* sf, int n_streams, const EncSched q, MbScratch& s, int stats, bool legacy_claim, Body body) {
  __shared__ BatchSlot s_slot[2];
  __shared__ int s_ids[2][ENC_WPC];
  __shared__ int s_fin[2];
  const int lane = threadIdx.x & 31, warp = threadIdx.x >> 5;
  const int mb_w = sf[0].p.mb_w, mb_h = sf[0].p.mb_h, n_mb = mb_w * mb_h, total = n_streams * n_mb;
  if (warp == ENC_WPC) {
    int p = 0, run_n = 0;
    for (;;) {
      if (lane == 0) {
        int k = 0, h = 0, n = 0;
        long long t_exposed = 0;
        bool exposed = false;
        unsigned long long n_poll = 0, n_fail = 0, n_idle = 0;
        for (;;) {
          const int fin = run_n ? *reinterpret_cast<volatile int*>(&s_fin[p ^ 1]) : 0;
          const bool all_done = fin >= run_n;
          if (stats && all_done && !exposed) { exposed = true; t_exposed = clock64(); }
          n_poll++;
          int c[2 * NQ + 1];
#pragma unroll
          for (int kk = 0; kk < NQ; kk++)
            asm volatile("ld.volatile.global.v2.s32 {%0, %1}, [%2];" : "=r"(c[kk]), "=r"(c[NQ + kk]) : "l"(ctl_head(q, kk)) : "memory");
          asm volatile("ld.volatile.global.s32 %0, [%1];" : "=r"(c[2 * NQ]) : "l"(ctl_done(q)) : "memory");
          if (c[2 * NQ] >= total) { n = -1; break; }
          int best = -1, best_avail = 0;
#pragma unroll
          for (int kk = NQ - 1; kk >= 0; kk--) {
            const int avail = c[NQ + kk] - c[kk];
            if (avail >= ENC_WPC && best_avail < ENC_WPC) { best = kk; best_avail = avail; }
            else if (best_avail < ENC_WPC && avail > best_avail) { best = kk; best_avail = avail; }
          }
          const bool full = best_avail >= ENC_WPC;
          const bool take = best >= 0 && (all_done || (!legacy_claim && full && (fin > 0 || best_avail >= 2 * ENC_WPC)));
          if (take) {
            int tail = 0;
#pragma unroll
            for (int kk = 0; kk < NQ; kk++) if (kk == best) { h = c[kk]; tail = c[NQ + kk]; }
            bool got = false;
            for (;;) {
              n = min(ENC_WPC, tail - h);
              if (n <= 0 || (n < ENC_WPC && !all_done)) break;
              const int old = atomicCAS(ctl_head(q, best), h, h + n);
              if (old == h) { got = true; break; }
              n_fail++;
              h = old;
            }
            if (got) { k = best; break; }
            __nanosleep(100 + 40 * (blockIdx.x & 7));
            continue;
          }
          n_idle++;
          __nanosleep(all_done ? 100 : fin > 0 ? 400 : 1500);
        }
        s_slot[p].k = k; s_slot[p].base = h; s_slot[p].n = n;
        s_fin[p] = 0;
        if (stats) {
          if (exposed) atomicAdd(&g_batch_stats[NQ][2], (unsigned long long)(clock64() - t_exposed));
          atomicAdd(&g_batch_stats[NQ][0], n_poll + (n_fail << 32));
          atomicAdd(&g_batch_stats[NQ][1], n_idle);
        }
      }
      __syncwarp();
      {
        const int kk = s_slot[p].k, nn = s_slot[p].n;
        if (lane < nn) {
          int id;
          while ((id = ld_volatile(q.queue + (size_t)kk * total + s_slot[p].base + lane)) < 0) {}
          s_ids[p][lane] = id;
        }
      }
      __syncwarp();
      enc_cta_barrier();
      run_n = s_slot[p].n;
      if (run_n < 0) break;
      p ^= 1;
    }
    return;
  }
  int p = 0, prev_k = -1, prev_n = 0;
  long long t_prev = 0;
  for (;;) {
    enc_cta_barrier();
    const int k = s_slot[p].k, n = s_slot[p].n;
    if (stats && threadIdx.x == 0) {
      const long long t = clock64();
      if (prev_k >= 0) {
        const unsigned long long dt = (unsigned long long)(t - t_prev);
        atomicAdd(&g_batch_stats[prev_k][0], 1ull);
        atomicAdd(&g_batch_stats[prev_k][1], (unsigned long long)prev_n);
        atomicAdd(&g_batch_stats[prev_k][2], dt);
        atomicAdd(&g_fill_stats[prev_k][min(prev_n, ENC_WPC)][0], 1ull);
        atomicAdd(&g_fill_stats[prev_k][min(prev_n, ENC_WPC)][1], dt);
      }
      t_prev = t; prev_k = k; prev_n = n;
    }
    if (n < 0) break;
    if (warp < n) {
      const long long t_task = stats ? clock64() : 0;
      const int id = s_ids[p][warp];
      run_task(sf, q, s, id, k + 1, mb_w, mb_h, total, n, body);
      if (lane == 0) atomicAdd(&s_fin[p], 1);
      if (stats && lane == 0) { atomicAdd(&g_task_wall[k][0], (unsigned long long)(clock64() - t_task)); atomicAdd(&g_task_wall[k][1], 1ull); }
    }
    p ^= 1;
  }
}

__global__ void k_esched_init(EncSched q, const StreamFrame* __restrict__ sf, int n_streams, int n_mb) {
  const int i = blockIdx.x * blockDim.x + threadIdx.x;
  if (i == 0) {
    int na = 0, ni = 0;
    const int total = n_streams * n_mb;
    for (int s = 0; s < n_streams; s++) {
      if (sf[s].p.is_idr) q.queue[(size_t)(MBS_I - 1) * total + ni++] = s * n_mb;
      else q.queue[(size_t)(MBS_A - 1) * total + na++] = s * n_mb;
    }
    for (int k = 0; k < kCtlInts; k++) q.ctl[k] = 0;
    *ctl_tail(q, MBS_A - 1) = na;
    *ctl_tail(q, MBS_I - 1) = ni;
  }
}

__global__ void k_sched_init(Sched q, int n_streams, int n_mb) {
  const int i = blockIdx.x * blockDim.x + threadIdx.x;
  if (i < n_streams) q.queue[i] = i * n_mb;
  if (i == 0) { *q.head = 0; *q.tail = n_streams; }
}

__device__ unsigned long long g_enc_stats[16];
#ifdef B2H264_PHASE_STATS
namespace mbk { __device__ unsigned long long g_phase[32]; }
extern "C" int b2h264_debug_phase_stats(unsigned long long* out32, int reset) {
  cudaError_t e = cudaMemcpyFromSymbol(out32, mbk::g_phase, sizeof(mbk::g_phase));
  if (e == cudaSuccess && reset) { unsigned long long z[32] = {0}; e = cudaMemcpyToSymbol(mbk::g_phase, z, sizeof(z)); }
  return (int)e;
}
#endif

#ifndef ENC_MIN_CTAS
#define ENC_MIN_CTAS 1
#endif
constexpr size_t kScratchSmem = sizeof(MbScratch) * DEC_WPC + 128;
static_assert(DEC_WPC >= ENC_WPC, "one scratch area size for both kernels");
__device__ __forceinline__ MbScratch& my_scratch(uint8_t* smem) {
  const uintptr_t a = (reinterpret_cast<uintptr_t>(smem) + 127) & ~uintptr_t(127);
  return reinterpret_cast<MbScratch*>(a)[threadIdx.x >> 5];
}

__global__ void __launch_bounds__(kEncThreads, ENC_MIN_CTAS) k_encode_mbs(const StreamFrame* __restrict__ sf, int n_streams, EncSched q, int stats,
                                                                          const __grid_constant__ CUtensorMap tm_ref, const void* tm_global,
                                                                          int win_mode ,
                                                                          int* started ) {
  extern __shared__ __align__(128) uint8_t smem[];
  if (threadIdx.x == 0 && started) *reinterpret_cast<volatile int*>(started) = 1;
  __shared__ WinBar s_wbar[ENC_WPC];
  MbScratch& s = my_scratch(smem);
  WinBar* wb = &s_wbar[min((int)(threadIdx.x >> 5), ENC_WPC - 1)];
  if ((threadIdx.x & 31) == 0 && threadIdx.x < 32 * ENC_WPC) {
    wb->phase = 0;
    asm volatile("mbarrier.init.shared::cta.b64 [%0], 1;" ::"r"((uint32_t)__cvta_generic_to_shared(&wb->bar)));
    asm volatile("fence.mbarrier_init.release.cluster;" ::: "memory");
  }
  __syncthreads();
  const void* tmap = win_mode == 1 ? (const void*)&tm_ref : win_mode == 3 ? tm_global : nullptr;
  const int wmode = win_mode == 3 ? 1 : win_mode;
  run_stages(sf, n_streams, q, s, stats & 1, (stats & 4) != 0, [&](const StreamFrame& F, int x, int y, int stage, int batch_n) {
    const long long t0 = (stats & 1) ? clock64() : 0;
    mb_ctx(s.ctx, F.p, F.f, x, y);
    if ((threadIdx.x & 31) == 0) { s.ctx.tmap_ref = tmap; s.ctx.wbar = wb; s.ctx.win_mode = wmode; s.ctx.batch_n = (stats & (stage == MBS_A ? 16 : 8)) ? batch_n : 0; s.ctx.batch_n_fine = (stats & 32) ? batch_n : 0; }
    __syncwarp();
    int next = mb_run_stage(s.ctx, s, stage);
    if (stats & 2) while (next != MBS_DONE) next = mb_run_stage(s.ctx, s, next);
    if ((stats & 1) && (threadIdx.x & 31) == 0) {
      atomicAdd(&g_enc_stats[2 * stage], (unsigned long long)(clock64() - t0));
      atomicAdd(&g_enc_stats[2 * stage + 1], 1ull);
    }
    return next;
  });
  if (threadIdx.x == 0 && started) reinterpret_cast<volatile int*>(started)[1] = 1;
}

#define DBK_WPC 8
#define DBK_CO_WPC 4
template <int WPC, int MIN_CTAS, bool BSL = false >
__global__ void __launch_bounds__(32 * WPC, MIN_CTAS) k_deblock_rows(const StreamFrame* __restrict__ sf, int n_streams, int* prog, int* counter,
                                                                      const int* enc_prog ,
                                                                      const int* enc_started ) {
  using Tile = typename std::conditional<BSL, DbkTileB, DbkTile>::type;
  __shared__ Tile tiles[WPC];
  if (enc_started != nullptr) {
    __shared__ int s_go;
    if (threadIdx.x == 0) {
      int go = 0;
      for (int i = 0; i < 300 && !(go = ld_volatile(enc_started)); i++) __nanosleep(1000);
      if (go && ld_volatile(enc_started + 1)) go = 0;
      s_go = go;
    }
    __syncthreads();
    if (!s_go) return;
  }
  Tile& t = tiles[threadIdx.x >> 5];
  const int lane = threadIdx.x & 31;
  const int mb_w = sf[0].p.mb_w, mb_h = sf[0].p.mb_h, units = n_streams * mb_h;
  for (;;) {
    int u = 0;
    if (lane == 0) u = atomicAdd(counter, 1);
    u = __shfl_sync(MBK_FULL, u, 0);
    if (u >= units) break;
    const int row = u / n_streams, si = u - row * n_streams;
    const StreamFrame& F = sf[si];
    int* mine = prog + si * mb_h + row;
    const int* up = mine - 1;
    const int* coded = enc_prog ? enc_prog + si * mb_h + (row + 1 < mb_h ? row + 1 : row) : nullptr;
    int seen = row > 0 ? 0 : mb_w, seen_enc = coded ? 0 : mb_w;
    for (int x = 0; x < mb_w; x++) {
      const int need = x + 2 < mb_w ? x + 2 : mb_w;
      if (seen < need || seen_enc < need) {
        if (lane == 0) {
          while (seen < need && (seen = ld_volatile(up)) < need) __nanosleep(40);
          while (seen_enc < need && (seen_enc = ld_volatile(coded)) < need) __nanosleep(200);
        }
        seen = __shfl_sync(MBK_FULL, seen, 0);
        seen_enc = __shfl_sync(MBK_FULL, seen_enc, 0);
        __threadfence();
      }
      deblock_one_mb_t<BSL>(F.p, F.f, x, row, t);
      __threadfence();
      __syncwarp();
      if (lane == 0) *reinterpret_cast<volatile int*>(mine) = x + 1;
    }
  }
}

__global__ void __launch_bounds__(32 * DEC_WPC) k_decode_mbs(const StreamFrame* __restrict__ sf, int n_streams, Sched q,
                                                            const MbOut* __restrict__ recs, const DecMbAux* __restrict__ aux) {
  extern __shared__ __align__(128) uint8_t smem[];
  MbScratch& s = my_scratch(smem);
  run_mbs(sf, n_streams, q, [&](const StreamFrame& F, int x, int y) {
    const int n_mb = F.p.mb_w * F.p.mb_h, si = (int)(&F - sf);
    const size_t r = (size_t)si * n_mb + y * F.p.mb_w + x;
    dec_one_mb(F.p, F.f, s, x, y, recs[r], aux[r]);
  });
}

__global__ void k_expand_lr_batch(const StreamFrame* __restrict__ sf) {
  const StreamFrame& F = sf[blockIdx.z / 3];
  const int pl = blockIdx.z % 3;
  const int pad = pl ? 16 : 32, st = pl ? F.p.rec_stride_c : F.p.rec_stride_y;
  const int w = (pl ? 8 : 16) * F.p.mb_w, h = (pl ? 8 : 16) * F.p.mb_h;
  const int y = blockIdx.x * blockDim.y + threadIdx.y;
  if (y >= h) return;
  uint8_t* row = F.f.rec[pl] + (size_t)y * st;
  const uint8_t l = row[0], r = row[w - 1];
  for (int x = threadIdx.x; x < pad; x += blockDim.x) { row[x - pad] = l; row[w + x] = r; }
}
__global__ void k_expand_tb_batch(const StreamFrame* __restrict__ sf) {
  const StreamFrame& F = sf[blockIdx.z / 3];
  const int pl = blockIdx.z % 3;
  const int pad = pl ? 16 : 32, st = pl ? F.p.rec_stride_c : F.p.rec_stride_y;
  const int w = (pl ? 8 : 16) * F.p.mb_w, h = (pl ? 8 : 16) * F.p.mb_h;
  const int x = blockIdx.x * blockDim.x + threadIdx.x - pad;
  if (x >= w + pad) return;
  uint8_t* pic = F.f.rec[pl];
  const uint8_t t = pic[x], b = pic[(size_t)(h - 1) * st + x];
  for (int y = 1 + blockIdx.y; y <= pad; y += gridDim.y) {
    pic[x - (ptrdiff_t)y * st] = t;
    pic[(size_t)(h - 1 + y) * st + x] = b;
  }
}

namespace mbk {
uint8_t h_alpha[52] = {0, 0, 0, 0, 0, 0, 0, 0, 0, 0, 0, 0, 0, 0, 0, 0, 4, 4, 5, 6, 7, 8, 9, 10, 12, 13, 15, 17, 20, 22, 25, 28,
                       32, 36, 40, 45, 50, 56, 63, 71, 80, 90, 101, 113, 127, 144, 162, 182, 203, 226, 255, 255};
uint8_t h_beta[52] = {0, 0, 0, 0, 0, 0, 0, 0, 0, 0, 0, 0, 0, 0, 0, 0, 2, 2, 2, 3, 3, 3, 3, 4, 4, 4, 6, 6, 7, 7, 8, 8,
                      9, 9, 10, 10, 11, 11, 12, 12, 13, 13, 14, 14, 15, 15, 16, 16, 17, 17, 18, 18};
uint8_t h_tc0[52][3] = {
    {0, 0, 0}, {0, 0, 0}, {0, 0, 0}, {0, 0, 0}, {0, 0, 0}, {0, 0, 0}, {0, 0, 0}, {0, 0, 0}, {0, 0, 0}, {0, 0, 0}, {0, 0, 0},
    {0, 0, 0}, {0, 0, 0}, {0, 0, 0}, {0, 0, 0}, {0, 0, 0}, {0, 0, 0}, {0, 0, 1}, {0, 0, 1}, {0, 0, 1}, {0, 0, 1}, {0, 1, 1},
    {0, 1, 1}, {1, 1, 1}, {1, 1, 1}, {1, 1, 1}, {1, 1, 1}, {1, 1, 2}, {1, 1, 2}, {1, 1, 2}, {1, 1, 2}, {1, 2, 3}, {1, 2, 3},
    {2, 2, 3}, {2, 2, 4}, {2, 3, 4}, {2, 3, 4}, {3, 3, 5}, {3, 4, 6}, {3, 4, 6}, {4, 5, 7}, {4, 5, 8}, {4, 6, 9}, {5, 7, 10},
    {6, 8, 11}, {6, 8, 13}, {7, 10, 14}, {8, 11, 16}, {9, 12, 18}, {10, 13, 20}, {11, 15, 23}, {13, 17, 25}};
}

int enc_upload_deblock_tables() {
  cudaError_t e;
  if ((e = cudaMemcpyToSymbol(mbk::c_alpha, mbk::h_alpha, sizeof(mbk::h_alpha))) != cudaSuccess) return (int)e;
  if ((e = cudaMemcpyToSymbol(mbk::c_beta, mbk::h_beta, sizeof(mbk::h_beta))) != cudaSuccess) return (int)e;
  if ((e = cudaMemcpyToSymbol(mbk::c_tc0, mbk::h_tc0, sizeof(mbk::h_tc0))) != cudaSuccess) return (int)e;
  return 0;
}

#include <mutex>
template <class K>
static int grid_blocks_for(K kernel, int threads, int* cache ) {
  static std::mutex mu;
  int dev = 0;
  cudaGetDevice(&dev);
  std::lock_guard<std::mutex> lock(mu);
  if (dev < 0 || dev >= 64) dev = 0;
  if (cache[dev]) return cache[dev];
  cudaFuncSetAttribute(kernel, cudaFuncAttributeMaxDynamicSharedMemorySize, (int)kScratchSmem);
  int sms = 0, per_sm = 0;
  cudaDeviceGetAttribute(&sms, cudaDevAttrMultiProcessorCount, dev);
  cudaOccupancyMaxActiveBlocksPerMultiprocessor(&per_sm, kernel, threads, kScratchSmem);
  if (per_sm < 1) per_sm = 1;
  return cache[dev] = sms * per_sm;
}
static int enc_grid_blocks() {
  static int cache[64];
  return grid_blocks_for(k_encode_mbs, kEncThreads, cache);
}
static int dec_grid_blocks() {
  static int cache[64];
  return grid_blocks_for(k_decode_mbs, 32 * DEC_WPC, cache);
}

static size_t enc_ctl_offset(size_t total) { return (32 + (3 + NQ) * total + 31) / 32 * 32; }
size_t enc_sched_ints(int n_streams, int n_mb) { return enc_ctl_offset((size_t)n_streams * n_mb) + kCtlInts + (size_t)n_streams * n_mb; }
size_t enc_stash_bytes(int n_streams, int mb_h) { return (size_t)n_streams * mb_h * kStashU4 * sizeof(uint4); }

static Sched make_sched(int* ws, int which, int total) {
  Sched q;
  q.head = ws + 2 * which; q.tail = ws + 2 * which + 1;
  (void)which;
  q.dep = ws + 32 + (size_t)total;
  q.queue = ws + 32 + (size_t)2 * total;
  return q;
}
static EncSched make_esched(int* ws, int total, void* stash) {
  EncSched q;
  q.ctl = ws + enc_ctl_offset((size_t)total);
  q.dep = ws + 32;
  q.queue = ws + 32 + (size_t)3 * total;
  q.stash = reinterpret_cast<uint4*>(stash);
  q.rowprog = nullptr;
  return q;
}

static int launch_deblock_rows(const StreamFrame* d_sf, int n_streams, int mb_h, int* prog, int* counter, const int* enc_prog, cudaStream_t st,
                               bool b_slices = false) {
  static int per_dev[64];
  int dev = 0, sms = 0;
  cudaGetDevice(&dev);
  if (dev < 0 || dev >= 64) dev = 0;
  if (!per_dev[dev]) {
    int per_sm = 0;
    cudaDeviceGetAttribute(&sms, cudaDevAttrMultiProcessorCount, dev);
    cudaOccupancyMaxActiveBlocksPerMultiprocessor(&per_sm, k_deblock_rows<DBK_WPC, 6>, 32 * DBK_WPC, 0);
    per_dev[dev] = sms * (per_sm < 1 ? 1 : per_sm);
  }
  const int units = n_streams * mb_h;
  int blocks = per_dev[dev];
  if (blocks > (units + DBK_WPC - 1) / DBK_WPC) blocks = (units + DBK_WPC - 1) / DBK_WPC;
  if (b_slices) k_deblock_rows<DBK_WPC, 6, true><<<blocks, 32 * DBK_WPC, 0, st>>>(d_sf, n_streams, prog, counter, enc_prog, nullptr);
  else k_deblock_rows<DBK_WPC, 6><<<blocks, 32 * DBK_WPC, 0, st>>>(d_sf, n_streams, prog, counter, enc_prog, nullptr);
  return b2h264_launched();
}
static int launch_deblock_rows_resident(const StreamFrame* d_sf, int n_streams, int mb_h, int* prog, int* counter, const int* enc_prog,
                                        const int* enc_started, cudaStream_t st) {
  int dev = 0, sms = 0;
  cudaGetDevice(&dev);
  cudaDeviceGetAttribute(&sms, cudaDevAttrMultiProcessorCount, dev);
  static bool carve_set[64];
  if (dev >= 0 && dev < 64 && !carve_set[dev]) {
    cudaFuncSetAttribute(k_deblock_rows<DBK_CO_WPC, 16>, cudaFuncAttributePreferredSharedMemoryCarveout, cudaSharedmemCarveoutMaxShared);
    carve_set[dev] = true;
  }
  const int units = n_streams * mb_h;
  int blocks = sms;
  if (blocks > (units + DBK_CO_WPC - 1) / DBK_CO_WPC) blocks = (units + DBK_CO_WPC - 1) / DBK_CO_WPC;
  k_deblock_rows<DBK_CO_WPC, 16><<<blocks, 32 * DBK_CO_WPC, 0, st>>>(d_sf, n_streams, prog, counter, enc_prog, enc_started);
  return b2h264_launched();
}

static int batch_sync_bits() {
  const char* v = getenv("B2H264_BATCH_SYNC");
  const int m = v ? atoi(v) : 1;
  return ((m & 1) ? 8 : 0) | ((m & 2) ? 16 : 0) | ((m & 4) ? 32 : 0);
}

int enc_launch_frame(const StreamFrame* d_sf, const uint8_t* const* d_src, int n_streams, int w, int h, int mb_w, int mb_h,
                     int* d_ws, void* d_stash, const void* tmap_ref, const void* d_tmap, int fast_mode, cudaStream_t st,
                     cudaStream_t st_dbk, cudaEvent_t ev_ready, cudaEvent_t ev_dbk) {
  int rc;
  if (d_src) {
    dim3 b(32, 8), g((mb_w * 4 + 31) / 32, (mb_h * 16 + 7) / 8, n_streams);
    k_pad_source<<<g, b, 0, st>>>(d_sf, d_src, w, h);
    if ((rc = b2h264_launched())) return rc;
  }
  if (fast_mode) {
    const int n_mb = mb_w * mb_h;
    k_vaa_sad8x8<<<dim3((n_mb + 7) / 8, n_streams), 256, 0, st>>>(d_sf, n_mb);
    if ((rc = b2h264_launched())) return rc;
  }
  const int total = n_streams * mb_w * mb_h;
  cudaMemsetAsync(d_ws + 32, 0, 2 * (size_t)total * sizeof(int), st);
  cudaMemsetAsync(d_ws + 32 + 2 * (size_t)total, 0xff, (size_t)(1 + NQ) * total * sizeof(int), st);
  EncSched qe = make_esched(d_ws, total, d_stash);
  int* dbk_prog = d_ws + 32 + (size_t)total;
  static const bool resident_dbk = getenv("B2H264_RESIDENT_DEBLOCK") != nullptr;
  const bool co = resident_dbk && st_dbk != nullptr;
  if (co) {
    qe.rowprog = d_ws + enc_ctl_offset((size_t)total) + kCtlInts;
    cudaMemsetAsync(qe.rowprog, 0, (size_t)n_streams * mb_h * sizeof(int), st);
  }
  k_esched_init<<<1, 32, 0, st>>>(qe, d_sf, n_streams, mb_w * mb_h);
  cudaMemsetAsync(d_ws + 2, 0, 3 * sizeof(int), st);
  int blocks = enc_grid_blocks();
  const int need = (total + ENC_WPC - 1) / ENC_WPC;
  if (blocks > need) blocks = need;
  static const int stats = (getenv("B2H264_ENC_STATS") ? 1 : 0) | (getenv("B2H264_FUSE_STAGES") ? 2 : 0) | (getenv("B2H264_LEGACY_CLAIM") ? 4 : 0) |
                           batch_sync_bits();
  CUtensorMap tm;
  memset(&tm, 0, sizeof(tm));
  static const int win_env = getenv("B2H264_ENC_WIN") ? atoi(getenv("B2H264_ENC_WIN")) : 1;
  int win_mode = win_env;
  if ((win_mode == 1 || win_mode == 3) && tmap_ref == nullptr) win_mode = 2;
  if (win_mode == 3 && d_tmap == nullptr) win_mode = 2;
  if (win_mode == 1) memcpy(&tm, tmap_ref, sizeof(tm));
  if (co && cudaEventRecord(ev_ready, st) != cudaSuccess) return (int)cudaGetLastError();
  k_encode_mbs<<<blocks, kEncThreads, kScratchSmem, st>>>(d_sf, n_streams, qe, stats, tm, d_tmap, win_mode, co ? d_ws + 3 : nullptr);
  if ((rc = b2h264_launched())) return rc;
  if (co) {
    if (cudaStreamWaitEvent(st_dbk, ev_ready, 0) != cudaSuccess) return (int)cudaGetLastError();
    if ((rc = launch_deblock_rows_resident(d_sf, n_streams, mb_h, dbk_prog, d_ws + 2, qe.rowprog, d_ws + 3, st_dbk))) return rc;
    if (cudaEventRecord(ev_dbk, st_dbk) != cudaSuccess) return (int)cudaGetLastError();
  }
  return 0;
}

int enc_launch_deblock_expand(const StreamFrame* d_sf, int n_streams, int mb_w, int mb_h, int* d_ws, cudaStream_t st, cudaEvent_t ev_dbk) {
  int rc;
  const int total = n_streams * mb_w * mb_h;
  int* dbk_prog = d_ws + 32 + (size_t)total;
  static const bool resident_dbk = getenv("B2H264_RESIDENT_DEBLOCK") != nullptr;
  if ((rc = launch_deblock_rows(d_sf, n_streams, mb_h, dbk_prog, d_ws + 2, resident_dbk ? d_ws + enc_ctl_offset((size_t)total) + kCtlInts : nullptr, st))) return rc;
  if (resident_dbk && ev_dbk && cudaStreamWaitEvent(st, ev_dbk, 0) != cudaSuccess) return (int)cudaGetLastError();
  k_expand_lr_batch<<<dim3((mb_h * 16 + 7) / 8, 1, 3 * n_streams), dim3(32, 8), 0, st>>>(d_sf);
  if ((rc = b2h264_launched())) return rc;
  k_expand_tb_batch<<<dim3((mb_w * 16 + 64 + 127) / 128, 4, 3 * n_streams), dim3(128), 0, st>>>(d_sf);
  return b2h264_launched();
}

size_t dec_sched_ints(int n_streams, int n_mb) { return 8 + 4 * (size_t)n_streams * n_mb; }
static Sched make_dec_sched(int* ws, int which, int total) {
  Sched q;
  q.head = ws + 2 * which; q.tail = ws + 2 * which + 1;
  q.dep = ws + 8 + (size_t)which * total;
  q.queue = ws + 8 + (size_t)(2 + which) * total;
  return q;
}
int dec_launch_frame(const StreamFrame* d_sf, int n_streams, int mb_w, int mb_h, int* d_ws, const MbOut* d_recs, const DecMbAux* d_aux, int deblock,
                     cudaStream_t st, int b_slices) {
  const int blocks_per_launch = dec_grid_blocks();
  int rc;
  const int total = n_streams * mb_w * mb_h;
  cudaMemsetAsync(d_ws + 8, 0, 2 * (size_t)total * sizeof(int), st);
  cudaMemsetAsync(d_ws + 8 + 2 * (size_t)total, 0xff, 2 * (size_t)total * sizeof(int), st);
  const Sched qc = make_dec_sched(d_ws, 0, total), qd = make_dec_sched(d_ws, 1, total);
  k_sched_init<<<(n_streams + 127) / 128, 128, 0, st>>>(qc, n_streams, mb_w * mb_h);
  k_sched_init<<<(n_streams + 127) / 128, 128, 0, st>>>(qd, n_streams, mb_w * mb_h);
  const int need = (total + DEC_WPC - 1) / DEC_WPC;
  k_decode_mbs<<<blocks_per_launch < need ? blocks_per_launch : need, 32 * DEC_WPC, kScratchSmem, st>>>(d_sf, n_streams, qc, d_recs, d_aux);
  if ((rc = b2h264_launched())) return rc;
  if (deblock) {
    cudaMemsetAsync(d_ws + 2, 0, sizeof(int), st);
    if ((rc = launch_deblock_rows(d_sf, n_streams, mb_h, d_ws + 8 + (size_t)total, d_ws + 2, nullptr, st, b_slices != 0))) return rc;
  }
  k_expand_lr_batch<<<dim3((mb_h * 16 + 7) / 8, 1, 3 * n_streams), dim3(32, 8), 0, st>>>(d_sf);
  if ((rc = b2h264_launched())) return rc;
  k_expand_tb_batch<<<dim3((mb_w * 16 + 64 + 127) / 128, 4, 3 * n_streams), dim3(128), 0, st>>>(d_sf);
  return b2h264_launched();
}

#define PACK_THREADS 256
__global__ void __launch_bounds__(PACK_THREADS) k_pack_records(const StreamFrame* __restrict__ sf, int n_mb, uint4* __restrict__ pack,
                                                               int32_t* __restrict__ idx, int32_t* __restrict__ cnt) {
  __shared__ int s_units;
  const int s = blockIdx.x, tid = threadIdx.x, lane = tid & 31, wi = tid >> 5;
  const MbOut* out = sf[s].f.out;
  int32_t* my_idx = idx + (size_t)s * n_mb;
  uint4* dst0 = pack + (size_t)s * n_mb * (sizeof(MbOut) / 16);
  if (tid == 0) s_units = 0;
  __syncthreads();
  for (int c0 = wi * 32; c0 < n_mb; c0 += PACK_THREADS) {
    const int mb = c0 + lane;
    const bool coded = mb < n_mb && out[mb].mb_type != MBT_PSKIP;
    unsigned m = __ballot_sync(0xffffffffu, coded);
    if (mb < n_mb && !coded) my_idx[mb] = -1;
    while (m) {
      const int j = __ffs(m) - 1;
      m &= m - 1;
      const MbOut* rec = out + c0 + j;
      const uint4* rq = reinterpret_cast<const uint4*>(rec);
      const int type = rec->mb_type, cbp = rec->cbp;
      uint4 a = make_uint4(0, 0, 0, 0), b = a;
      bool want = false;
      if (lane < 16) want = type == MBT_I16x16 ? (cbp & 15) != 0 : ((cbp >> (lane >> 2)) & 1) != 0;
      else if (lane < 24) want = (cbp >> 4) == 2;
      if (want) {
        const int q = lane < 16 ? 7 + 2 * lane : 40 + 2 * (lane - 16);
        a = rq[q]; b = rq[q + 1];
        want = (a.x | a.y | a.z | a.w | b.x | b.y | b.z | b.w) != 0;
      }
      const unsigned mask = __ballot_sync(0xffffffffu, want);
      int off = 0;
      if (lane == 0) off = atomicAdd(&s_units, 4 + __popc(mask));
      off = __shfl_sync(0xffffffffu, off, 0);
      uint4* dst = dst0 + (size_t)off * 2;
      if (lane < 8) {
        uint4 v = rq[lane < 7 ? lane : 39];
        if (lane == 0) v.y = (v.y & 0xffu) | (mask << 8);
        dst[lane] = v;
      }
      if (want) {
        const int pos = 8 + 2 * __popc(mask & ((1u << lane) - 1));
        dst[pos] = a; dst[pos + 1] = b;
      }
      if (lane == 0) my_idx[c0 + j] = off;
    }
  }
  __syncthreads();
  if (tid == 0) cnt[s] = s_units;
}

int enc_launch_pack(const StreamFrame* d_sf, int n_streams, int n_mb, MbOut* pack, int32_t* idx, int32_t* cnt, cudaStream_t st) {
  static_assert(sizeof(MbOut) == 896 && offsetof(MbOut, luma) == 112 && offsetof(MbOut, chroma_dc) == 624 && offsetof(MbOut, chroma_ac) == 640 &&
                offsetof(MbOut, pad0) == 5, "compact record layout");
  k_pack_records<<<n_streams, PACK_THREADS, 0, st>>>(d_sf, n_mb, reinterpret_cast<uint4*>(pack), idx, cnt);
  return b2h264_launched();
}

__global__ void __launch_bounds__(256) k_unpack_records(const uint4* __restrict__ pack, size_t stream_stride_u4, const int32_t* __restrict__ idx,
                                                        MbOut* __restrict__ recs, int n_mb) {
  const int s = blockIdx.y, lane = threadIdx.x & 31, mb = blockIdx.x * 8 + (threadIdx.x >> 5);
  if (mb >= n_mb) return;
  const int32_t o = idx[(size_t)s * n_mb + mb];
  uint4* dst = reinterpret_cast<uint4*>(recs + (size_t)s * n_mb + mb);
  const uint4 z = make_uint4(0, 0, 0, 0);
  if (o < 0) {
    if (lane < 7) dst[lane] = lane == 0 ? make_uint4((uint32_t)MBT_PSKIP | ((uint32_t)(-1 - o) << 16), 0, 0, 0) : z;
    else if (lane == 7) dst[39] = z;
    return;
  }
  const uint4* src = pack + (size_t)s * stream_stride_u4 + (size_t)o * 2;
  const uint32_t mask = src[0].y >> 8;
  if (lane < 7) {
    uint4 v = src[lane];
    if (lane == 0) v.y &= 0xffu;
    dst[lane] = v;
  } else if (lane == 7) {
    dst[39] = src[7];
  } else {
    const int b = lane - 8, q = b < 16 ? 7 + 2 * b : 40 + 2 * (b - 16);
    uint4 v0 = z, v1 = z;
    if ((mask >> b) & 1) { const int pos = 8 + 2 * __popc(mask & ((1u << b) - 1)); v0 = src[pos]; v1 = src[pos + 1]; }
    dst[q] = v0; dst[q + 1] = v1;
  }
}
int dec_launch_unpack(const void* d_pack, size_t stream_stride_bytes, const int32_t* d_idx, MbOut* d_recs, int n_streams, int n_mb, cudaStream_t st) {
  k_unpack_records<<<dim3((n_mb + 7) / 8, n_streams), 256, 0, st>>>(reinterpret_cast<const uint4*>(d_pack), stream_stride_bytes / 16, d_idx, d_recs, n_mb);
  return b2h264_launched();
}

size_t enc_scratch_bytes() { return sizeof(MbScratch); }

extern "C" int b2h264_debug_enc_stats(unsigned long long* out16, int reset) {
  cudaError_t e = cudaMemcpyFromSymbol(out16, g_enc_stats, sizeof(g_enc_stats));
  if (e != cudaSuccess) return (int)e;
  if (reset) { unsigned long long z[16] = {0}; e = cudaMemcpyToSymbol(g_enc_stats, z, sizeof(z)); }
  return (int)e;
}
```

openh264_b200/csrc/enc_launch.h:

```cpp
#pragma once
#include <cuda_runtime.h>
#include <stddef.h>

#include "enc_types.h"

struct StreamFrame {
  EncFrameParams p;
  EncFramePtrs f;
};

int enc_upload_deblock_tables();
int enc_launch_frame(const StreamFrame* d_sf, const uint8_t* const* d_src, int n_streams, int w, int h, int mb_w, int mb_h,
                     int* d_sched_ws, void* d_stash, const void* tmap_ref ,
                     const void* d_tmap ,
                     int fast_mode , cudaStream_t st,
                     cudaStream_t st_dbk ,
                     cudaEvent_t ev_ready, cudaEvent_t ev_dbk );
int enc_launch_deblock_expand(const StreamFrame* d_sf, int n_streams, int mb_w, int mb_h, int* d_sched_ws, cudaStream_t st,
                              cudaEvent_t ev_dbk );
size_t enc_sched_ints(int n_streams, int n_mb);
size_t enc_stash_bytes(int n_streams, int mb_h);
size_t enc_scratch_bytes();
size_t dec_sched_ints(int n_streams, int n_mb);
int dec_launch_frame(const StreamFrame* d_sf, int n_streams, int mb_w, int mb_h, int* d_ws, const MbOut* d_recs, const DecMbAux* d_aux, int deblock,
                     cudaStream_t st, int b_slices );
int dec_launch_unpack(const void* d_pack, size_t stream_stride_bytes, const int32_t* d_idx, MbOut* d_recs, int n_streams, int n_mb, cudaStream_t st);
int enc_launch_pack(const StreamFrame* d_sf, int n_streams, int n_mb, MbOut* pack, int32_t* idx, int32_t* cnt, cudaStream_t st);
```

openh264_b200/csrc/enc_mb.cuh:

```cuda
#pragma once
#include <stddef.h>

#include "enc_intra.cuh"
#include "enc_types.h"

namespace mbk {

struct WinBar { unsigned long long bar; uint32_t phase; uint32_t pad; };

struct MbCtx {
  EncFrameParams p;
  EncFramePtrs f;
  int mbx, mby, nb;
  int qp, qp_c, lambda;
  const void* tmap_ref;
  WinBar* wbar;
  int win_mode;
  int batch_n;
  int batch_n_fine;
};

struct MeState {
  int mv_x, mv_y;
  int mvp_x, mvp_y;
  uint32_t sad_cost, satd_cost;
  int satd;
  const uint8_t* ref;
};

struct InterState {
  int32_t is_skip, cost_luma, cost_skip_mb, p16_mvx, p16_mvy, final_type, cost16, bb;
};

enum { WIN_W = 64, WIN_H = 48 };

struct alignas(128) MbScratch {
  RecTile tile;
  InterState st;
  int16_t mvc[30][2];
  int8_t  refc[30];
  int8_t  i4m[25];
  int8_t  skip_flag[4];
  int32_t sadc[4];
  int32_t sad_skip[4];
  MbInfo  info;
  MbInfo  nbi[4];
  int32_t nb_sad[4];
  int32_t nb_skip_sad[4];
  alignas(16) MbOut out;
  alignas(16) uint8_t pred_y[2][256];
  alignas(128) uint8_t pred_c[2][128];
  uint8_t skip_pred[384];
  uint8_t qplane[3][18 * 32];
  int16_t coef[384];
  alignas(16) uint8_t cur_y[256];
  uint8_t cur_c[128];
  int16_t dc16[16];
  int32_t red[32];
  MbCtx ctx;
  MeState me[9];
  int16_t mvcand[5][2];
  int32_t win_x0, win_y0, win_ok;
  uint32_t t_last;
};
static_assert(offsetof(MbScratch, skip_pred) == offsetof(MbScratch, pred_c) + 256 &&
              offsetof(MbScratch, qplane) == offsetof(MbScratch, skip_pred) + 384 && offsetof(MbScratch, coef) == offsetof(MbScratch, qplane) + 3 * 18 * 32 &&
              256 + 384 + 3 * 18 * 32 + 768 >= WIN_W * WIN_H,
              "pred_c / skip_pred / qplane / coef double as the search window");
static_assert(offsetof(MbScratch, pred_c) % 128 == 0 && offsetof(MbScratch, skip_pred) % 16 == 0 && offsetof(MbScratch, pred_y) % 16 == 0 &&
              offsetof(MbScratch, out) % 16 == 0, "alignment of the parked ranges / the bulk copy destination");
constexpr int kParkCore = (int)((offsetof(MbScratch, out) + 4 * MBOUT_HEADER_WORDS + 15) / 16 * 16);
constexpr int kParkExtra = 512;
constexpr int kParkSlot = kParkCore + kParkExtra;
MBK_HD uint8_t* scratch_win(MbScratch& s) { return &s.pred_c[0][0]; }

#if defined(B2H264_PHASE_STATS) && defined(__CUDA_ARCH__)
extern __device__ unsigned long long g_phase[32];
__device__ __forceinline__ void phase_mark(MbScratch& s, int i) {
  if ((threadIdx.x & 31) == 0) { const uint32_t t = (uint32_t)clock(); atomicAdd(&g_phase[i], (unsigned long long)(uint32_t)(t - s.t_last)); s.t_last = t; }
}
#else
MBK_HD void phase_mark(MbScratch&, int) {}
#endif


MBK_HD int blk_x(int k) { return (k & 1) | ((k >> 1) & 2); }
MBK_HD int blk_y(int k) { return ((k >> 1) & 1) | ((k >> 2) & 2); }
MBK_HD int blk_raster(int k) { return blk_y(k) * 4 + blk_x(k); }

MBK_HD uint8_t ld_cg_u8(const uint8_t* p) {
#ifdef __CUDA_ARCH__
  return __ldcg(p);
#else
  return *p;
#endif
}

MBK_HD uint32_t ld_cg_u32(const uint32_t* p) {
#ifdef __CUDA_ARCH__
  return __ldcg(p);
#else
  return *p;
#endif
}

MBK_HD void mb_load_neighbors(const MbCtx& c, MbScratch& s) {
  const int mbw = c.p.mb_w, idx = c.mby * mbw + c.mbx;
  const int offs[4] = {-mbw - 1, -mbw, -mbw + 1, -1};
  const int bits[4] = {NB_TOPLEFT, NB_TOP, NB_TOPRIGHT, NB_LEFT};
  for (int i = lane_id(); i < 4 * (int)(sizeof(MbInfo) / 4); i += MBK_WS) {
    const int k = i / (int)(sizeof(MbInfo) / 4), w = i - k * (int)(sizeof(MbInfo) / 4);
    if (c.nb & bits[k])
      reinterpret_cast<uint32_t*>(&s.nbi[k])[w] = ld_cg_u32(reinterpret_cast<const uint32_t*>(c.f.mbi + idx + offs[k]) + w);
  }
  for (int k = lane_id(); k < 8; k += MBK_WS) {
    const int j = k & 3;
    const bool av = (c.nb & bits[j]) != 0;
    if (k < 4) s.nb_sad[j] = av ? (int32_t)ld_cg_u32(reinterpret_cast<const uint32_t*>(c.f.sad_cost + idx + offs[j])) : 0;
    else s.nb_skip_sad[j] = av ? (int32_t)ld_cg_u32(reinterpret_cast<const uint32_t*>(&c.f.rec_info[idx + offs[j]].skip_sad)) : 0;
  }
  warp_sync();
}

MBK_HD void mb_load_cur(const MbCtx& c, MbScratch& s) {
  const uint8_t* y = c.f.cur[0] + (size_t)(c.mby * 16) * c.p.cur_stride_y + c.mbx * 16;
  for (int i = lane_id(); i < 64; i += MBK_WS) {
    const int r = i >> 2, c4 = (i & 3) << 2;
    *reinterpret_cast<uint32_t*>(s.cur_y + r * 16 + c4) = *reinterpret_cast<const uint32_t*>(y + (size_t)r * c.p.cur_stride_y + c4);
  }
  for (int i = lane_id(); i < 32; i += MBK_WS) {
    const int pl = i >> 4, r = (i >> 1) & 7, c4 = (i & 1) << 2;
    const uint8_t* src = c.f.cur[1 + pl] + (size_t)(c.mby * 8 + r) * c.p.cur_stride_c + c.mbx * 8 + c4;
    *reinterpret_cast<uint32_t*>(s.cur_c + pl * 64 + r * 8 + c4) = *reinterpret_cast<const uint32_t*>(src);
  }
  warp_sync();
}

MBK_HD void mb_load_borders(const MbCtx& c, MbScratch& s) {
  RecTile& t = s.tile;
  const uint8_t* ry = c.f.rec[0] + (ptrdiff_t)(c.mby * 16 - 1) * c.p.rec_stride_y + c.mbx * 16;
  const uint8_t* ru = c.f.rec[1] + (ptrdiff_t)(c.mby * 8 - 1) * c.p.rec_stride_c + c.mbx * 8;
  const uint8_t* rv = c.f.rec[2] + (ptrdiff_t)(c.mby * 8 - 1) * c.p.rec_stride_c + c.mbx * 8;
  for (int i = lane_id(); i < 43 + 32; i += MBK_WS) {
    if (i < 25) {
      const int x = i - 1;
      const bool ok = x < 0 ? (c.nb & NB_TOPLEFT) : x < 16 ? (c.nb & NB_TOP) : (c.nb & NB_TOPRIGHT);
      *tile_y(t, x, -1) = ok ? ld_cg_u8(ry + x) : 0;
    } else if (i < 34) {
      const int x = i - 26;
      const bool ok = x < 0 ? (c.nb & NB_TOPLEFT) : (c.nb & NB_TOP);
      *tile_c(t.u, x, -1) = ok ? ld_cg_u8(ru + x) : 0;
    } else if (i < 43) {
      const int x = i - 35;
      const bool ok = x < 0 ? (c.nb & NB_TOPLEFT) : (c.nb & NB_TOP);
      *tile_c(t.v, x, -1) = ok ? ld_cg_u8(rv + x) : 0;
    } else {
      const int j = i - 43;
      const bool ok = (c.nb & NB_LEFT) != 0;
      if (j < 16) *tile_y(t, -1, j) = ok ? ld_cg_u8(ry + (ptrdiff_t)(j + 1) * c.p.rec_stride_y - 1) : 0;
      else if (j < 24) *tile_c(t.u, -1, j - 16) = ok ? ld_cg_u8(ru + (ptrdiff_t)(j - 15) * c.p.rec_stride_c - 1) : 0;
      else *tile_c(t.v, -1, j - 24) = ok ? ld_cg_u8(rv + (ptrdiff_t)(j - 23) * c.p.rec_stride_c - 1) : 0;
    }
  }
  warp_sync();
}

MBK_STAGE void mb_load_all(const MbCtx& c, MbScratch& s) {
  const int mbw = c.p.mb_w, idx = c.mby * mbw + c.mbx, l = lane_id();
  constexpr int kW = (int)(sizeof(MbInfo) / 4);
#ifdef __CUDA_ARCH__
  auto nb_off = [&](int k) { return k == 3 ? -1 : -mbw - 1 + k; };
  auto nb_bit = [](int k) { return (int)((((uint32_t)NB_TOPLEFT) | ((uint32_t)NB_TOP << 8) | ((uint32_t)NB_TOPRIGHT << 16) | ((uint32_t)NB_LEFT << 24)) >> (8 * k)) & 0xff; };
  uint32_t nbw[4];
#pragma unroll
  for (int r = 0; r < 4; r++) {
    const int i = l + 32 * r, k = i / kW, w = i - k * kW;
    nbw[r] = (i < 4 * kW && (c.nb & nb_bit(k & 3))) ? ld_cg_u32(reinterpret_cast<const uint32_t*>(c.f.mbi + idx + nb_off(k & 3)) + w) : 0u;
  }
  uint32_t hist = 0;
  if (l < 8 && (c.nb & nb_bit(l & 3)))
    hist = l < 4 ? ld_cg_u32(reinterpret_cast<const uint32_t*>(c.f.sad_cost + idx + nb_off(l & 3)))
                 : ld_cg_u32(reinterpret_cast<const uint32_t*>(&c.f.rec_info[idx + nb_off(l & 3)].skip_sad));
  const uint8_t* cy = c.f.cur[0] + (size_t)(c.mby * 16) * c.p.cur_stride_y + c.mbx * 16;
  const uint32_t cy0 = *reinterpret_cast<const uint32_t*>(cy + (size_t)(l >> 2) * c.p.cur_stride_y + ((l & 3) << 2));
  const uint32_t cy1 = *reinterpret_cast<const uint32_t*>(cy + (size_t)(8 + (l >> 2)) * c.p.cur_stride_y + ((l & 3) << 2));
  const uint32_t cc = *reinterpret_cast<const uint32_t*>(c.f.cur[1 + (l >> 4)] + (size_t)(c.mby * 8 + ((l >> 1) & 7)) * c.p.cur_stride_c +
                                                          c.mbx * 8 + ((l & 1) << 2));
  const uint8_t* ry = c.f.rec[0] + (ptrdiff_t)(c.mby * 16 - 1) * c.p.rec_stride_y + c.mbx * 16;
  const uint8_t* ru = c.f.rec[1] + (ptrdiff_t)(c.mby * 8 - 1) * c.p.rec_stride_c + c.mbx * 8;
  const uint8_t* rv = c.f.rec[2] + (ptrdiff_t)(c.mby * 8 - 1) * c.p.rec_stride_c + c.mbx * 8;
  uint8_t tb[2] = {0, 0};
#pragma unroll
  for (int r = 0; r < 2; r++) {
    const int i = l + 32 * r;
    if (i < 25) {
      const int x = i - 1;
      if (x < 0 ? (c.nb & NB_TOPLEFT) : x < 16 ? (c.nb & NB_TOP) : (c.nb & NB_TOPRIGHT)) tb[r] = ld_cg_u8(ry + x);
    } else if (i < 34) {
      const int x = i - 26;
      if (x < 0 ? (c.nb & NB_TOPLEFT) : (c.nb & NB_TOP)) tb[r] = ld_cg_u8(ru + x);
    } else if (i < 43) {
      const int x = i - 35;
      if (x < 0 ? (c.nb & NB_TOPLEFT) : (c.nb & NB_TOP)) tb[r] = ld_cg_u8(rv + x);
    }
  }
  uint8_t lb = 0;
  if (c.nb & NB_LEFT)
    lb = l < 16 ? ld_cg_u8(ry + (ptrdiff_t)(l + 1) * c.p.rec_stride_y - 1)
                : l < 24 ? ld_cg_u8(ru + (ptrdiff_t)(l - 15) * c.p.rec_stride_c - 1) : ld_cg_u8(rv + (ptrdiff_t)(l - 23) * c.p.rec_stride_c - 1);
#pragma unroll
  for (int r = 0; r < 4; r++) {
    const int i = l + 32 * r;
    if (i < 4 * kW) reinterpret_cast<uint32_t*>(&s.nbi[0])[i] = nbw[r];
  }
  if (l < 4) s.nb_sad[l] = (int32_t)hist;
  else if (l < 8) s.nb_skip_sad[l - 4] = (int32_t)hist;
  *reinterpret_cast<uint32_t*>(s.cur_y + (l >> 2) * 16 + ((l & 3) << 2)) = cy0;
  *reinterpret_cast<uint32_t*>(s.cur_y + (8 + (l >> 2)) * 16 + ((l & 3) << 2)) = cy1;
  *reinterpret_cast<uint32_t*>(s.cur_c + (l >> 4) * 64 + ((l >> 1) & 7) * 8 + ((l & 1) << 2)) = cc;
  RecTile& t = s.tile;
#pragma unroll
  for (int r = 0; r < 2; r++) {
    const int i = l + 32 * r;
    if (i < 25) *tile_y(t, i - 1, -1) = tb[r];
    else if (i < 34) *tile_c(t.u, i - 26, -1) = tb[r];
    else if (i < 43) *tile_c(t.v, i - 35, -1) = tb[r];
  }
  if (l < 16) *tile_y(t, -1, l) = lb;
  else if (l < 24) *tile_c(t.u, -1, l - 16) = lb;
  else *tile_c(t.v, -1, l - 24) = lb;
  warp_sync();
#else
  (void)idx; (void)l;
  mb_load_neighbors(c, s);
  mb_load_cur(c, s);
  mb_load_borders(c, s);
#endif
}

MBK_HD void mb_store_recon_skip(const MbCtx& c, MbScratch& s) {
  uint8_t* ry = c.f.rec[0] + (size_t)(c.mby * 16) * c.p.rec_stride_y + c.mbx * 16;
  for (int i = lane_id(); i < 64; i += MBK_WS) {
    const int r = i >> 2, c4 = (i & 3) << 2;
    *reinterpret_cast<uint32_t*>(ry + (size_t)r * c.p.rec_stride_y + c4) = *reinterpret_cast<const uint32_t*>(s.skip_pred + r * 16 + c4);
  }
  for (int i = lane_id(); i < 32; i += MBK_WS) {
    const int pl = i >> 4, r = (i >> 1) & 7, c4 = (i & 1) << 2;
    uint8_t* dst = c.f.rec[1 + pl] + (size_t)(c.mby * 8 + r) * c.p.rec_stride_c + c.mbx * 8 + c4;
    *reinterpret_cast<uint32_t*>(dst) = *reinterpret_cast<const uint32_t*>(s.skip_pred + 256 + 64 * pl + r * 8 + c4);
  }
  warp_sync();
}

MBK_STAGE void mb_store_recon(const MbCtx& c, MbScratch& s) {
  uint8_t* ry = c.f.rec[0] + (size_t)(c.mby * 16) * c.p.rec_stride_y + c.mbx * 16;
  for (int i = lane_id(); i < 64; i += MBK_WS) {
    const int r = i >> 2, c4 = (i & 3) << 2;
    const uint8_t* src = tile_y(s.tile, c4, r);
    *reinterpret_cast<uint32_t*>(ry + (size_t)r * c.p.rec_stride_y + c4) =
        (uint32_t)src[0] | ((uint32_t)src[1] << 8) | ((uint32_t)src[2] << 16) | ((uint32_t)src[3] << 24);
  }
  for (int i = lane_id(); i < 32; i += MBK_WS) {
    const int pl = i >> 4, r = (i >> 1) & 7, c4 = (i & 1) << 2;
    const uint8_t* src = tile_c(pl ? s.tile.v : s.tile.u, c4, r);
    uint8_t* dst = c.f.rec[1 + pl] + (size_t)(c.mby * 8 + r) * c.p.rec_stride_c + c.mbx * 8 + c4;
    *reinterpret_cast<uint32_t*>(dst) = (uint32_t)src[0] | ((uint32_t)src[1] << 8) | ((uint32_t)src[2] << 16) | ((uint32_t)src[3] << 24);
  }
  warp_sync();
}

MBK_HD int md_i16x16_inl(const MbCtx& c, MbScratch& s, int* best_buf) {
  int modes[4] = {0, 0, 0, 0};
  const int n = i16_modes(c.nb & 7, modes);
  const uint32_t packed = (uint32_t)modes[0] | ((uint32_t)modes[1] << 8) | ((uint32_t)modes[2] << 16) | ((uint32_t)modes[3] << 24);
  int best = 0x7fffffff, best_mode = modes[0], bb = 1;
  const uint8_t* org = tile_y(s.tile, 0, 0);
  MBK_NO_UNROLL
  for (int i = 0; i < n; i++) {
    const int mode = (int)((packed >> (8 * i)) & 0xffu);
    uint8_t* dst = s.pred_y[1 - bb];
    pred_i16(dst, org, TY_PITCH, mode);
    const int cost = (c.p.fast_mode ? warp_sad(dst, 16, s.cur_y, 16, 4, 4) : warp_satd(dst, 16, s.cur_y, 16, 4, 4)) +
                     c.lambda * ue_bits(map_i16(mode));
    if (cost < best) { best = cost; best_mode = mode; bb = 1 - bb; }
    warp_sync();
  }
  s.out.i16_mode = (uint8_t)map_i16(best_mode);
  *best_buf = bb;
  return best;
}
MBK_FN int md_i16x16(const MbCtx& c, MbScratch& s, int* best_buf) { return md_i16x16_inl(c, s, best_buf); }

MBK_FN int md_chroma(const MbCtx& c, MbScratch& s, int* best_buf) {
  int modes[4];
  const int n = chroma_modes(c.nb & 7, modes);
  int best = 0x7fffffff, best_mode = modes[0], bb = 1;
  for (int i = 0; i < n; i++) {
    uint8_t* dst = s.pred_c[1 - bb];
    pred_chroma(dst, tile_c(s.tile.u, 0, 0), TC_PITCH, modes[i]);
    pred_chroma(dst + 64, tile_c(s.tile.v, 0, 0), TC_PITCH, modes[i]);
    const int cost = (c.p.fast_mode ? warp_sad(dst, 8, s.cur_c, 8, 3, 3) + warp_sad(dst + 64, 8, s.cur_c + 64, 8, 3, 3)
                                     : warp_satd(dst, 8, s.cur_c, 8, 3, 3) + warp_satd(dst + 64, 8, s.cur_c + 64, 8, 3, 3)) +
                     c.lambda * ue_bits(map_chroma(modes[i]));
    if (cost < best) { best = cost; best_mode = modes[i]; bb = 1 - bb; }
    warp_sync();
  }
  s.out.chroma_mode = (uint8_t)map_chroma(best_mode);
  *best_buf = bb;
  return best;
}

MBK_FN void enc_rec_i16x16(const MbCtx& c, MbScratch& s, const uint8_t* pred) {
  const int qp = c.qp;
  const int16_t* ff = tbl_quant_ff(qp + 6);
  const int16_t* mf = tbl_quant_mf(qp);
  for (int k = lane_id(); k < 16; k += MBK_WS) {
    int16_t d[16];
    const int o = blk_y(k) * 4 * 16 + blk_x(k) * 4;
    dct4x4(d, s.cur_y + o, 16, pred + o, 16);
    for (int i = 0; i < 16; i++) s.coef[16 * k + i] = d[i];
  }
  warp_sync();
  int16_t dcq[16];
  {
    int16_t in[16];
    for (int k = 0; k < 16; k++) in[k] = s.coef[16 * k];
    hadamard_t4_dc(dcq, in);
    quant4x4_dc(dcq, ff[0] << 1, mf[0] >> 1);
  }
  int16_t lv[16];
  scan4x4_dcac(lv, dcq);
  const int n_dc = nonzero_count(lv);
  for (int i = lane_id(); i < 16; i += MBK_WS) s.out.luma_dc[i] = lv[i];
  int nz_ac = 0;
  for (int k = lane_id(); k < 16; k += MBK_WS) {
    int16_t d[16], l[16];
    for (int i = 0; i < 16; i++) d[i] = s.coef[16 * k + i];
    quant4x4(d, ff, mf);
    scan4x4_ac(l, d);
    const int nz = nonzero_count(l);
    for (int i = 0; i < 16; i++) { s.coef[16 * k + i] = d[i]; s.out.luma[k][i] = l[i]; }
    s.info.nnz[blk_raster(k)] = (int8_t)nz;
    nz_ac += nz;
  }
  nz_ac = warp_sum(nz_ac);
  if (n_dc > 0) {
    if (qp < 12) { ihadamard4x4(dcq); dequant_luma_dc4x4(dcq, qp); }
    else dequant_ihadamard4x4(dcq, (uint16_t)(tbl_dequant(qp)[0] >> 2));
  }
  warp_sync();
  uint8_t* rec = tile_y(s.tile, 0, 0);
  if (nz_ac > 0) {
    s.info.cbp = 15;
    for (int k = lane_id(); k < 16; k += MBK_WS) {
      int16_t d[16];
      for (int i = 0; i < 16; i++) d[i] = s.coef[16 * k + i];
      dequant4x4(d, tbl_dequant(qp));
      d[0] = dcq[blk_raster(k)];
      const int o = blk_y(k) * 4, ox = blk_x(k) * 4;
      idct4x4_rec(rec + o * TY_PITCH + ox, TY_PITCH, pred + o * 16 + ox, 16, d);
    }
  } else if (n_dc > 0) {
    for (int i = lane_id(); i < 256; i += MBK_WS) {
      const int y = i >> 4, x = i & 15;
      rec[y * TY_PITCH + x] = (uint8_t)clip255(pred[i] + ((dcq[(y & 12) + (x >> 2)] + 32) >> 6));
    }
  } else {
    for (int i = lane_id(); i < 256; i += MBK_WS) rec[(i >> 4) * TY_PITCH + (i & 15)] = pred[i];
  }
  warp_sync();
}

MBK_FN int md_enc_i4x4(const MbCtx& c, MbScratch& s, int cost_limit) {
  const int qp = c.qp;
  const int16_t* ff = tbl_quant_ff(qp + 6);
  const int16_t* mf = tbl_quant_mf(qp);
  const int lam4 = c.lambda << 2, lam1 = c.lambda;
  int total = 0;
  for (int k = 0; k < 16; k++) {
    const int bx = blk_x(k), by = blk_y(k);
    uint8_t* org = tile_y(s.tile, bx * 4, by * 4);
    const uint8_t* cur = s.cur_y + by * 4 * 16 + bx * 4;
    const int lm = s.i4m[(by + 1) * 5 + bx], tm = s.i4m[by * 5 + bx + 1];
    const int pm = (lm == -1 || tm == -1) ? 2 : (lm < tm ? lm : tm);
    int modes[9];
    const int n = i4_modes(i4_avail(c.nb, k), modes);
    int best_cost, best_mode;
    if (!c.p.fast_mode) {
      int key = 0x7fffffff;
      for (int j = lane_id(); j < n; j += MBK_WS) {
        uint8_t p[16];
        pred_i4(p, org, TY_PITCH, modes[j]);
        const int cost = satd4x4_pred(p, cur, 16) + (pm == map_i4(modes[j]) ? lam1 : lam4);
        const int kj = (cost << 4) | j;
        if (kj < key) key = kj;
      }
      key = warp_min(key);
      best_cost = key >> 4; best_mode = modes[key & 15];
    } else {
      for (int j = lane_id(); j < n; j += MBK_WS) {
        uint8_t p[16];
        pred_i4(p, org, TY_PITCH, modes[j]);
        int sad = 0;
        for (int q = 0; q < 16; q++) sad += iabs((int)p[q] - (int)cur[(q >> 2) * 16 + (q & 3)]);
        s.red[modes[j]] = sad + (pm == map_i4(modes[j]) ? lam1 : lam4);
      }
      warp_sync();
      const int32_t* cst = s.red;
      if (n == 9 || n == 7) {
        best_mode = I4_DC; best_cost = cst[I4_DC];
        const int cH = cst[I4_H], cV = cst[I4_V];
        if (cH < best_cost) { best_cost = cH; best_mode = I4_H; }
        if (cV < best_cost) { best_cost = cV; best_mode = I4_V; }
#define I4_TRY(m) do { if (cst[m] < best_cost) { best_cost = cst[m]; best_mode = (m); } } while (0)
        if (cV < cH) {
          if (n == 9) {
            I4_TRY(I4_VR); I4_TRY(I4_VL);
            if (cst[I4_VR] < cV || cst[I4_VL] < cV) {
              if (cst[I4_VR] < cst[I4_VL]) I4_TRY(I4_DDR); else I4_TRY(I4_DDL);
            }
          } else { I4_TRY(I4_DDR); I4_TRY(I4_VR); }
        } else {
          I4_TRY(I4_HD); I4_TRY(I4_HU);
          if (cst[I4_HD] < cH || cst[I4_HU] < cH) {
            if (cst[I4_HD] < cst[I4_HU]) I4_TRY(I4_DDR);
            else if (n == 9) I4_TRY(I4_DDL);
          }
        }
#undef I4_TRY
      } else {
        best_cost = 0x7fffffff; best_mode = modes[0];
        for (int j = 0; j < n; j++) if (cst[modes[j]] < best_cost) { best_cost = cst[modes[j]]; best_mode = modes[j]; }
      }
      warp_sync();
    }
    total += best_cost;
    if (total >= cost_limit) break;
    const int fm = map_i4(best_mode);
    s.out.prev_i4_flag[k] = (int8_t)(pm == fm);
    s.out.rem_i4_mode[k] = (int8_t)(fm < pm ? fm : fm - 1);
    s.i4m[(by + 1) * 5 + bx + 1] = (int8_t)fm;
    s.info.i4_mode[by * 4 + bx] = (int8_t)fm;
    if (lane_id() == 0) {
      uint8_t p[16];
      int16_t d[16], l[16];
      pred_i4(p, org, TY_PITCH, best_mode);
      dct4x4(d, cur, 16, p, 4);
      quant4x4(d, ff, mf);
      scan4x4_dcac(l, d);
      const int nz = nonzero_count(l);
      for (int i = 0; i < 16; i++) s.out.luma[k][i] = l[i];
      s.info.nnz[by * 4 + bx] = (int8_t)nz;
      if (nz > 0) {
        s.info.cbp |= (uint8_t)(1 << (k >> 2));
        dequant4x4(d, tbl_dequant(qp));
        idct4x4_rec(org, TY_PITCH, p, 4, d);
      } else {
        for (int i = 0; i < 16; i++) org[(i >> 2) * TY_PITCH + (i & 3)] = p[i];
      }
    }
    warp_sync();
  }
  return total + 24 * c.lambda;
}

MBK_FN void enc_rec_uv(const MbCtx& c, MbScratch& s, int uv, bool inter) {
  int16_t* res = s.coef + 256 + 64 * uv;
  const int qpc = c.qp_c;
  const int16_t* ff = tbl_quant_ff(qpc + (inter ? 0 : 6));
  const int16_t* mf = tbl_quant_mf(qpc);
  const int16_t dcin[4] = {res[0], res[16], res[32], res[48]};
  int16_t dc[4];
  const int nz_dc = hadamard_quant2x2(dcin, (int16_t)(ff[0] << 1), (int16_t)(mf[0] >> 1), dc);
  warp_sync();
  for (int j = lane_id(); j < 4; j += MBK_WS) {
    int16_t d[16], l[16];
    for (int i = 0; i < 16; i++) d[i] = res[16 * j + i];
    d[0] = 0;
    const int16_t mx = quant4x4_max(d, ff, mf);
    if (mx == 0) { for (int i = 0; i < 16; i++) l[i] = 0; }
    else scan4x4_ac(l, d);
    for (int i = 0; i < 16; i++) { res[16 * j + i] = d[i]; s.out.chroma_ac[4 * uv + j][i] = l[i]; }
    s.red[j] = mx;
    s.red[4 + j] = mx == 0 ? 0 : single_ctr4x4(l);
    s.red[8 + j] = nonzero_count(l);
  }
  if (lane_id() == 0) for (int i = 0; i < 4; i++) s.out.chroma_dc[uv][i] = dc[i];
  warp_sync();
  int ctr = 0;
  for (int j = 0; j < 4; j++) {
    const int mx = s.red[j];
    if (mx == 0) continue;
    if (inter) {
      if (mx > 1) ctr += 9;
      else if (ctr < 7) ctr += s.red[4 + j];
    } else ctr = 0x7fffffff;
  }
  if (ctr < 7) {
    for (int i = lane_id(); i < 64; i += MBK_WS) res[i] = 0;
    if (lane_id() == 0) for (int j = 0; j < 4; j++) s.info.nnz[16 + 4 * uv + j] = 0;
  } else {
    for (int j = lane_id(); j < 4; j += MBK_WS) {
      s.info.nnz[16 + 4 * uv + j] = (int8_t)s.red[8 + j];
      int16_t d[16];
      for (int i = 0; i < 16; i++) d[i] = res[16 * j + i];
      dequant4x4(d, tbl_dequant(qpc));
      for (int i = 0; i < 16; i++) res[16 * j + i] = d[i];
    }
    if (lane_id() == 0) s.info.cbp = (uint8_t)((s.info.cbp & 0x0F) | 0x20);
  }
  warp_sync();
  if (nz_dc > 0 && lane_id() == 0) {
    dequant_ihadamard2x2_dc(dc, tbl_dequant(qpc)[0]);
    if (2 != (s.info.cbp >> 4)) s.info.cbp |= 0x10;
    res[0] = dc[0]; res[16] = dc[1]; res[32] = dc[2]; res[48] = dc[3];
  }
  warp_sync();
}

MBK_FN void dct_chroma(MbScratch& s, const uint8_t* pred) {
  for (int t = lane_id(); t < 8; t += MBK_WS) {
    const int uv = t >> 2, j = t & 3, ox = (j & 1) * 4, oy = (j >> 1) * 4;
    int16_t d[16];
    dct4x4(d, s.cur_c + 64 * uv + oy * 8 + ox, 8, pred + 64 * uv + oy * 8 + ox, 8);
    for (int i = 0; i < 16; i++) s.coef[256 + 64 * uv + 16 * j + i] = d[i];
  }
  warp_sync();
}
MBK_FN void rec_chroma(MbScratch& s, const uint8_t* pred) {
  for (int t = lane_id(); t < 8; t += MBK_WS) {
    const int uv = t >> 2, j = t & 3, ox = (j & 1) * 4, oy = (j >> 1) * 4;
    int16_t d[16];
    for (int i = 0; i < 16; i++) d[i] = s.coef[256 + 64 * uv + 16 * j + i];
    idct4x4_rec(tile_c(uv ? s.tile.v : s.tile.u, ox, oy), TC_PITCH, pred + 64 * uv + oy * 8 + ox, 8, d);
  }
  warp_sync();
}

MBK_FN void fill_i4_cache(const MbCtx& c, MbScratch& s) {
  if (lane_id() == 0) {
    for (int i = 0; i < 25; i++) s.i4m[i] = -1;
    if (c.nb & NB_LEFT) {
      const MbInfo* l = &s.nbi[3];
      for (int y = 0; y < 4; y++) s.i4m[(y + 1) * 5] = l->mb_type == MBT_I4x4 ? l->i4_mode[y * 4 + 3] : 2;
    }
    if (c.nb & NB_TOP) {
      const MbInfo* t = &s.nbi[1];
      for (int x = 0; x < 4; x++) s.i4m[x + 1] = t->mb_type == MBT_I4x4 ? t->i4_mode[12 + x] : 2;
    }
  }
  warp_sync();
}

MBK_FN bool intra_try_i4x4(const MbCtx& c, MbScratch& s) {
  if (!c.p.fast_mode) return true;
  int sum = 0, sqr = 0;
  for (int k = lane_id(); k < 16; k += MBK_WS) {
    const uint8_t* p = s.cur_y + (k >> 2) * 4 * 16 + (k & 3) * 4;
    int a = 0;
    for (int q = 0; q < 16; q++) a += p[(q >> 2) * 16 + (q & 3)];
    a >>= 4;
    sum += a; sqr += a * a;
  }
  sum = warp_sum(sum); sqr = warp_sum(sqr);
  return sqr - ((sum * sum) >> 4) >= 150;
}

MBK_FN int intra_mb_md_enc(const MbCtx& c, MbScratch& s, int cost_limit_for_i16 ) {
  (void)cost_limit_for_i16;
  int bb;
  int cost = md_i16x16(c, s, &bb);
  bool use_i4 = false;
  if (lane_id() == 0) { s.info.mb_type = MBT_I16x16; s.info.cbp = 0; }
  warp_sync();
  fill_i4_cache(c, s);
  if (intra_try_i4x4(c, s)) {
    const int cost4 = md_enc_i4x4(c, s, cost);
    if (cost4 < cost) { use_i4 = true; cost = cost4; if (lane_id() == 0) s.info.mb_type = MBT_I4x4; warp_sync(); }
  }
  if (!use_i4) {
    if (lane_id() == 0) s.info.cbp = 0;
    warp_sync();
    enc_rec_i16x16(c, s, s.pred_y[bb]);
  }
  int cb;
  md_chroma(c, s, &cb);
  dct_chroma(s, s.pred_c[cb]);
  enc_rec_uv(c, s, 0, false);
  enc_rec_uv(c, s, 1, false);
  rec_chroma(s, s.pred_c[cb]);
  return cost;
}

MBK_STAGE void mb_publish(const MbCtx& c, MbScratch& s) {
  const int idx = c.mby * c.p.mb_w + c.mbx;
  if (lane_id() == 0) {
    s.info.qp = (uint8_t)c.qp; s.info.qp_c = (uint8_t)c.qp_c;
    s.out.mb_type = s.info.mb_type; s.out.cbp = s.info.cbp; s.out.qp = (uint8_t)c.qp;
    for (int i = 0; i < 24; i++) s.out.nnz[i] = s.info.nnz[i];
  }
  warp_sync();
  const uint32_t* si = reinterpret_cast<const uint32_t*>(&s.info);
  uint32_t* di = reinterpret_cast<uint32_t*>(c.f.mbi + idx);
  for (int i = lane_id(); i < (int)(sizeof(MbInfo) / 4); i += MBK_WS) di[i] = si[i];
  const uint32_t* so = reinterpret_cast<const uint32_t*>(&s.out);
  uint32_t* dout = reinterpret_cast<uint32_t*>(c.f.out + idx);
  const int n_out = s.info.mb_type == MBT_PSKIP ? MBOUT_HEADER_WORDS : (int)(sizeof(MbOut) / 4);
  for (int i = lane_id(); i < n_out; i += MBK_WS) dout[i] = so[i];
  warp_sync();
}

}
```

openh264_b200/csrc/enc_types.h:

```cpp
#pragma once
#include <stdint.h>

enum {
  MBT_I4x4 = 0, MBT_I16x16 = 1, MBT_P16x16 = 2, MBT_P16x8 = 3, MBT_P8x16 = 4, MBT_P8x8 = 5, MBT_PSKIP = 6,
  MBT_IPCM = 7,
  MBT_B = 8, MBT_BSKIP = 9
};
#define MBT_IS_INTRA(t) ((t) <= MBT_I16x16 || (t) == MBT_IPCM)
#define MBT_IS_B(t) ((t) == MBT_B || (t) == MBT_BSKIP)
#define MBT_IS_INTER(t) (((t) >= MBT_P16x16 && (t) <= MBT_PSKIP) || MBT_IS_B(t))

typedef struct {
  int16_t mv[16][2];
  int8_t  nnz[24];
  int8_t  i4_mode[16];
  int16_t p16x16_mv[2];
  int32_t sad_cost;
  uint8_t mb_type;
  uint8_t cbp;
  uint8_t qp, qp_c;
  int8_t  ref_idx;
  uint8_t t8x8;
  uint8_t pad[2];
} MbInfo;

typedef struct {
  int16_t mv16[2];
  int32_t skip_sad;
  uint8_t mb_type;
  uint8_t pad[3];
} RefMbInfo;

typedef struct {
  uint8_t mb_type, cbp, qp, i16_mode;
  uint8_t chroma_mode;
  uint8_t pad0[3];
  int8_t  prev_i4_flag[16];
  int8_t  rem_i4_mode[16];
  int16_t mvd[4][2];
  int8_t  nnz[24];
  int16_t luma_dc[16];
  int16_t luma[16][16];
  int16_t chroma_dc[2][4];
  int16_t chroma_ac[8][16];
} MbOut;
typedef struct {
  uint8_t avail;
  uint8_t flags;
  uint8_t dbk_idc;
  int8_t  alpha_off, beta_off;
  uint8_t pad;
  uint16_t slice;
  uint8_t sub_type[4];
  int8_t  ref_idx[4];
  int16_t mvd[16][2];
} DecMbAux;
typedef struct {
  int8_t  ref_idx[4];
  uint8_t pred_lists[4];
  int16_t w1[4];
  int16_t mv[16][2];
  uint8_t wp_on;
  uint8_t wp_log2[2];
  uint8_t pad;
  int16_t wp[4][3][2];
} DecMbAuxB;
#define DECAUX_SUB 1
#define DECAUX_CIP 2
#define DECAUX_T8 4

#define MBOUT_HEADER_WORDS 20

typedef struct {
  int32_t mb_w, mb_h;
  int32_t cur_stride_y, cur_stride_c;
  int32_t rec_stride_y, rec_stride_c;
  int32_t qp;
  int32_t is_idr;
  int32_t mv_range;
  int32_t ref_is_p;
  int32_t ref_plane;
  int32_t dec_mode;
  int32_t fast_mode;
  int32_t dbk_idc, dbk_off_a, dbk_off_b;
  int32_t dec_cqp_off;
} EncFrameParams;

typedef struct {
  const uint8_t* cur[3];
  uint8_t* rec[3];
  const uint8_t* ref[3];
  MbInfo* mbi;
  RefMbInfo* rec_info;
  const RefMbInfo* ref_info;
  MbOut* out;
  int32_t* sad_cost;
  const int32_t* vaa_sad8x8;
  const uint8_t* dpb0[3];
  int64_t dpb_stride;
  const DecMbAux* dec_aux;
  const DecMbAuxB* dec_aux_b;
  const uint8_t* prev_luma;
  int32_t* mb_bits;
} EncFramePtrs;
```

Measured before the change: 4601.

## Add parallel P-skip prepass kernel that speculatively evaluates skip per macroblock

Adds a fully parallel prepass kernel that evaluates P-skip at a guessed motion vector (co-located reference MV) for every macroblock. It stores the SAD, cost and quantisation verdict in a SkipRec and writes the skip reconstruction directly. The wavefront-ordered main encode kernel then reuses the record when the real predicted skip MV matches, skipping motion compensation, DCT and recon stores for those blocks. The cost is an extra kernel launch, extra memory traffic, and wasted prepass work wherever the guessed MV misses.

```diff
diff --git a/openh264_b200/csrc/enc_batch.cu b/openh264_b200/csrc/enc_batch.cu
--- a/openh264_b200/csrc/enc_batch.cu
+++ b/openh264_b200/csrc/enc_batch.cu
@@ -3,6 +3,7 @@
 #include <condition_variable>
 #include <functional>
 #include <mutex>
+#include <stdlib.h>
 #include <string.h>
 #include <thread>
 #include <vector>
@@ -48,6 +49,7 @@
   int32_t* d_sad = nullptr;
   int32_t* d_prog = nullptr;
   int32_t* d_bits = nullptr;
+  SkipRec* d_skip = nullptr;
   bool mb_bits_on = false;
   int* d_tickets = nullptr;
   void* d_stash = nullptr;
@@ -163,6 +165,7 @@
   CK(cudaMemset(e->d_sad, 0, S * e->n_mb * sizeof(int32_t)));
   CK(cudaMalloc(&e->d_prog, S * 2 * mbh * sizeof(int32_t)));
   CK(cudaMalloc(&e->d_bits, S * e->n_mb * sizeof(int32_t)));
+  CK(cudaMalloc(&e->d_skip, S * e->n_mb * sizeof(SkipRec)));
   CK(cudaMalloc(&e->d_tickets, enc_sched_ints((int)S, e->n_mb) * sizeof(int)));
   CK(cudaMalloc(&e->d_stash, enc_stash_bytes((int)S, e->ctl[0].sp.mb_h)));
   e->bs.resize(S);
@@ -178,7 +181,7 @@
   cudaSetDevice(e->cfg.device);
   cudaStreamSynchronize(e->st);
   delete e->pool;
-  cudaFree(e->d_pic_all); cudaFree(e->d_cur); cudaFree(e->d_vaa); cudaFree(e->d_tmap); cudaFree(e->d_src); cudaFree(e->d_mbi); cudaFree(e->d_sad); cudaFree(e->d_prog); cudaFree(e->d_bits); cudaFree(e->d_tickets); cudaFree(e->d_stash);
+  cudaFree(e->d_pic_all); cudaFree(e->d_cur); cudaFree(e->d_vaa); cudaFree(e->d_tmap); cudaFree(e->d_src); cudaFree(e->d_mbi); cudaFree(e->d_sad); cudaFree(e->d_prog); cudaFree(e->d_bits); cudaFree(e->d_skip); cudaFree(e->d_tickets); cudaFree(e->d_stash);
   cudaFreeHost(e->h_src);
   for (int i = 0; i < 2; i++) {
     cudaFree(e->d_rinfo[i]); cudaFree(e->d_out[i]); cudaFree(e->d_sf[i]); cudaFree(e->d_srcptr[i]);
@@ -223,6 +226,9 @@
     }
     CK(cudaMemcpyAsync(dd, from, e->frame_bytes, cudaMemcpyHostToDevice, e->st_in));
   }
+  const char* pp_env = getenv("B2H264_SKIP_PREPASS");
+  const int prepass = pp_env ? atoi(pp_env) : 1;
+  bool any_p = false;
   sl.idr.assign(S, 0);
   for (int i = 0; i < n; i++) {
     const int s = sl.act[i];
@@ -245,6 +251,8 @@
     F.f.out = e->d_out[k] + (size_t)i * e->n_mb;
     F.f.sad_cost = e->d_sad + (size_t)s * e->n_mb;
     F.f.mb_bits = e->mb_bits_on ? e->d_bits + (size_t)s * e->n_mb : nullptr;
+    F.f.skip_rec = prepass && !idr ? e->d_skip + (size_t)s * e->n_mb : nullptr;
+    any_p = any_p || !idr;
     e->idr_next[s] = 0;
     e->have_ref_p[s] = !idr;
   }
@@ -257,7 +265,7 @@
   CK(cudaMemcpyAsync(e->d_srcptr[k], e->h_srcptr[k], n * sizeof(uint8_t*), cudaMemcpyHostToDevice, e->st));
   CK(cudaEventRecord(sl.ev0, e->st));
   int rc = enc_launch_frame(e->d_sf[k], e->d_srcptr[k], n, e->cfg.width, e->cfg.height, mbw, mbh, e->d_tickets, e->d_stash,
-                            e->have_tmap ? e->tmap_pic : nullptr, e->d_tmap, e->cfg.complexity_low != 0, e->st, e->st_dbk, sl.ev_ready, sl.ev_dbk);
+                            e->have_tmap ? e->tmap_pic : nullptr, e->d_tmap, e->cfg.complexity_low != 0, prepass && any_p ? prepass : 0, e->st, e->st_dbk, sl.ev_ready, sl.ev_dbk);
   if (rc) return rc;
   CK(cudaEventRecord(sl.ev1, e->st));
   rc = enc_launch_deblock_expand(e->d_sf[k], n, mbw, mbh, e->d_tickets, e->st, sl.ev_dbk);
diff --git a/openh264_b200/csrc/enc_frame.cuh b/openh264_b200/csrc/enc_frame.cuh
--- a/openh264_b200/csrc/enc_frame.cuh
+++ b/openh264_b200/csrc/enc_frame.cuh
@@ -57,7 +57,7 @@
   warp_sync();
   if (next == MBS_DONE) {
     phase_mark(s, 10);
-    if (s.info.mb_type == MBT_PSKIP && s.st.is_skip != 0) mb_store_recon_skip(c, s);
+    if (s.info.mb_type == MBT_PSKIP && s.st.is_skip != 0) { if (s.st.is_skip == 1) mb_store_recon_skip(c, s); }
     else mb_store_recon(c, s);
     mb_publish(c, s);
     if (c.f.mb_bits != nullptr) {
diff --git a/openh264_b200/csrc/enc_inter.cuh b/openh264_b200/csrc/enc_inter.cuh
--- a/openh264_b200/csrc/enc_inter.cuh
+++ b/openh264_b200/csrc/enc_inter.cuh
@@ -142,9 +142,10 @@
   warp_sync();
 }
 
-struct SkipResult { bool ok; int cost_luma; int cost_skip; int mvx, mvy; };
-
-MBK_STAGE bool try_py_skip(const MbCtx& c, MbScratch& s) {
+struct SkipEval { bool in_range, quant_ok, ok; int sad_y, sad_mb, cost_luma; };
+
+template <class Scratch>
+MBK_STAGE bool try_py_skip(const MbCtx& c, Scratch& s) {
   const int16_t* ff = tbl_quant_ff(c.qp);
   const int16_t* mf = tbl_quant_mf(c.qp);
   int big = 0, ctr = 0;
@@ -158,7 +159,8 @@
   big = warp_sum(big); ctr = warp_sum(ctr);
   return big == 0 && ctr < 6;
 }
-MBK_STAGE bool try_puv_skip(const MbCtx& c, MbScratch& s, int uv) {
+template <class Scratch>
+MBK_STAGE bool try_puv_skip(const MbCtx& c, Scratch& s, int uv) {
   const int16_t* res = s.coef + 256 + 64 * uv;
   const int16_t* ff = tbl_quant_ff(c.qp_c);
   const int16_t* mf = tbl_quant_mf(c.qp_c);
@@ -175,7 +177,8 @@
   big = warp_sum(big); ctr = warp_sum(ctr);
   return !dc_fail && big == 0 && ctr < 7;
 }
-MBK_FN void dct_luma_mb(MbScratch& s, const uint8_t* pred ) {
+template <class Scratch>
+MBK_FN void dct_luma_mb(Scratch& s, const uint8_t* pred ) {
   for (int k = lane_id(); k < 16; k += MBK_WS) {
     int16_t d[16];
     const int o = blk_y(k) * 4 * 16 + blk_x(k) * 4;
@@ -185,22 +188,24 @@
   warp_sync();
 }
 
-MBK_STAGE SkipResult pskip_enc(const MbCtx& c, MbScratch& s, int sad_pred_skip, int ref_mb_type) {
-  SkipResult r;
-  r.ok = false; r.cost_luma = 0; r.cost_skip = 0;
-  int mvx, mvy;
-  pred_skip_mv(s, &mvx, &mvy);
-  r.mvx = mvx; r.mvy = mvy;
+MBK_HD bool skip_sad_rule(const MbCtx& c, int sad_mb, int sad_pred_skip, int ref_mb_type) {
+  return sad_mb == 0 || sad_mb < sad_pred_skip ||
+         (c.p.ref_is_p && ref_mb_type == MBT_PSKIP && sad_mb < c.f.ref_info[c.mby * c.p.mb_w + c.mbx].skip_sad);
+}
+
+template <class Scratch>
+MBK_HD SkipEval skip_eval_at(const MbCtx& c, Scratch& s, int mvx, int mvy, bool speculative, int sad_pred_skip, int ref_mb_type) {
+  SkipEval e;
+  e.in_range = false; e.quant_ok = false; e.ok = false; e.sad_y = 0; e.sad_mb = 0; e.cost_luma = 0;
   const int ix = mvx >> 2, iy = mvy >> 2;
   int n = c.mbx * 16 + ix;
-  if (n < -29 || n > c.p.mb_w * 16 + 12) return r;
+  if (n < -29 || n > c.p.mb_w * 16 + 12) return e;
   n = c.mby * 16 + iy;
-  if (n < -29 || n > c.p.mb_h * 16 + 12) return r;
+  if (n < -29 || n > c.p.mb_h * 16 + 12) return e;
+  e.in_range = true;
   uint8_t* py = s.skip_pred;
-  phase_mark(s, 12);
   warp_mc_luma(ref_luma(c, ix, iy), c.p.rec_stride_y, py, 16, mvx, mvy, 16, 16);
   warp_sync();
-  phase_mark(s, 13);
   const int sad_y = warp_sad(s.cur_y, 16, py, 16, 4, 4);
   MBK_NO_UNROLL
   for (int pl = 0; pl < 2; pl++)
@@ -208,10 +213,9 @@
   warp_sync();
   const int sad_c = warp_sad(s.cur_c, 8, s.skip_pred + 256, 8, 3, 3) + warp_sad(s.cur_c + 64, 8, s.skip_pred + 320, 8, 3, 3);
   const int sad_mb = sad_y + sad_c;
-  phase_mark(s, 14);
-  bool ok = sad_mb == 0 || sad_mb < sad_pred_skip ||
-            (c.p.ref_is_p && ref_mb_type == MBT_PSKIP && sad_mb < c.f.ref_info[c.mby * c.p.mb_w + c.mbx].skip_sad);
-  if (!ok) {
+  e.sad_y = sad_y; e.sad_mb = sad_mb;
+  const bool sad_ok = !speculative && skip_sad_rule(c, sad_mb, sad_pred_skip, ref_mb_type);
+  if (!sad_ok) {
     dct_luma_mb(s, py);
     if (try_py_skip(c, s)) {
       for (int t = lane_id(); t < 4; t += MBK_WS) {
@@ -235,22 +239,49 @@
         }
         uv_ok = try_puv_skip(c, s, uv);
       }
-      ok = uv_ok;
-    }
-  }
+      e.quant_ok = uv_ok;
+    }
+  }
+  e.ok = sad_ok || e.quant_ok;
+  if (speculative || e.ok)
+    e.cost_luma = c.p.fast_mode ? sad_y : warp_satd_inl(s.cur_y, 16, py, 16, 4, 4);
+  return e;
+}
+
+MBK_HD bool skip_result(const MbCtx& c, MbScratch& s, bool ok, int sad_y, int sad_mb, int cost_luma) {
+  if (ok && lane_id() == 0) {
+    s.st.cost_luma = cost_luma;
+    s.st.cost_skip_mb = sad_mb;
+    if (c.p.fast_mode) c.f.sad_cost[c.mby * c.p.mb_w + c.mbx] = sad_y;
+  }
+  return ok;
+}
+
+MBK_STAGE bool pskip_enc(const MbCtx& c, MbScratch& s, int mvx, int mvy, int sad_pred_skip, int ref_mb_type) {
+  phase_mark(s, 12);
+  const SkipEval e = skip_eval_at(c, s, mvx, mvy, false, sad_pred_skip, ref_mb_type);
   phase_mark(s, 15);
-  if (ok) {
-    r.ok = true;
-    if (c.p.fast_mode) {
-      r.cost_luma = sad_y;
-      if (lane_id() == 0) c.f.sad_cost[c.mby * c.p.mb_w + c.mbx] = sad_y;
-    } else {
-      r.cost_luma = warp_satd_inl(s.cur_y, 16, py, 16, 4, 4);
-    }
-    phase_mark(s, 16);
-    r.cost_skip = sad_mb;
-  }
-  return r;
+  return skip_result(c, s, e.ok, e.sad_y, e.sad_mb, e.cost_luma);
+}
+
+template <class Scratch>
+MBK_HD void skip_prepass_mb(const MbCtx& c, Scratch& s, bool force_miss) {
+  const int idx = c.mby * c.p.mb_w + c.mbx;
+  int mvx = 0, mvy = 0;
+  if (c.p.ref_is_p) { mvx = c.f.ref_info[idx].mv16[0]; mvy = c.f.ref_info[idx].mv16[1]; }
+  if (force_miss) mvx += 1;
+  mb_load_cur(c, s);
+  const SkipEval e = skip_eval_at(c, s, mvx, mvy, true, 0, 0xff);
+  if (e.in_range) mb_store_recon_skip(c, s);
+  if (lane_id() == 0) {
+    SkipRec r;
+    r.mv[0] = (int16_t)(force_miss ? -32768 : mvx); r.mv[1] = (int16_t)mvy;
+    r.sad_mb = e.sad_mb; r.cost_luma = e.cost_luma; r.sad_y = (uint16_t)e.sad_y;
+    r.flags = (uint8_t)((e.quant_ok ? SKIPREC_QUANT_OK : 0) | (e.in_range ? 0 : SKIPREC_OUT_OF_RANGE));
+    r.pad = 0;
+    c.f.skip_rec[idx] = r;
+  }
+  warp_sync();
 }
 
 MBK_HD void win_issue(const MbCtx& c, MbScratch& s, int sx, int sy) {
@@ -578,20 +609,32 @@
   const bool keep_skip = sk_l && sk_t && sk_tr;
   int cost_luma = 0, cost_skip_mb = 0;
   bool is_skip = false;
-  if ((c.p.ref_is_p && ref_mb_type == MBT_PSKIP) || try_skip) {
-    const SkipResult r = pskip_enc(c, s, predict_sad_skip(s), ref_mb_type);
-    if (r.ok) {
-      is_skip = true;
-      cost_luma = r.cost_luma; cost_skip_mb = r.cost_skip;
-      p16_mvx = r.mvx; p16_mvy = r.mvy;
-      mb_mv_set(s, 0, 4, 4, r.mvx, r.mvy);
-    }
+  const bool skip_test = (c.p.ref_is_p && ref_mb_type == MBT_PSKIP) || try_skip;
+  const bool prepass = c.f.skip_rec != nullptr;
+  int mvx = 0, mvy = 0;
+  bool hit = false, hit_ok = false;
+  if (skip_test) {
+    pred_skip_mv(s, &mvx, &mvy);
+    hit = prepass && s.skrec.mv[0] == mvx && s.skrec.mv[1] == mvy;
+    if (hit) hit_ok = (s.skrec.flags & SKIPREC_OUT_OF_RANGE) == 0 &&
+                      (skip_sad_rule(c, s.skrec.sad_mb, predict_sad_skip(s), ref_mb_type) || (s.skrec.flags & SKIPREC_QUANT_OK) != 0);
+  }
+  const bool done_by_prepass = hit_ok && keep_skip;
+  if (hit_ok && !keep_skip) mb_load_skip_pred(c, s);
+  if (hit) is_skip = skip_result(c, s, hit_ok, s.skrec.sad_y, s.skrec.sad_mb, s.skrec.cost_luma);
+  else if (skip_test) is_skip = pskip_enc(c, s, mvx, mvy, predict_sad_skip(s), ref_mb_type);
+  if (lane_id() == 0) s.skip_hit = !(prepass && skip_test) ? 0 : hit ? 1 : 2;
+  warp_sync();
+  if (is_skip) {
+    cost_luma = s.st.cost_luma; cost_skip_mb = s.st.cost_skip_mb;
+    p16_mvx = mvx; p16_mvy = mvy;
+    mb_mv_set(s, 0, 4, 4, mvx, mvy);
   }
   mbk_batch_sync(6, c.batch_n);
   phase_mark(s, 2);
   if (is_skip && keep_skip) {
     decided_pskip(c, s);
-    st_save(s, 1, cost_luma, cost_skip_mb, p16_mvx, p16_mvy, MBT_PSKIP);
+    st_save(s, done_by_prepass ? 2 : 1, cost_luma, cost_skip_mb, p16_mvx, p16_mvy, MBT_PSKIP);
     inter_tail(c, s);
     return MBS_DONE;
   }
diff --git a/openh264_b200/csrc/enc_kernels.cu b/openh264_b200/csrc/enc_kernels.cu
--- a/openh264_b200/csrc/enc_kernels.cu
+++ b/openh264_b200/csrc/enc_kernels.cu
@@ -66,6 +66,17 @@
   v += __shfl_xor_sync(0xffffffffu, v, 4);
   v += __shfl_xor_sync(0xffffffffu, v, 8);
   if ((lane & 14) == 0) const_cast<int32_t*>(F.f.vaa_sad8x8)[(size_t)mb * 4 + (lane >> 4) * 2 + (lane & 1)] = v;
+}
+
+#define SKIP_PP_WPC 8
+__global__ void __launch_bounds__(32 * SKIP_PP_WPC, 3) k_skip_prepass(const StreamFrame* __restrict__ sf, int n_mb, int force_miss) {
+  __shared__ SkipScratch scr[SKIP_PP_WPC];
+  const StreamFrame& F = sf[blockIdx.y];
+  const int mb = blockIdx.x * SKIP_PP_WPC + (threadIdx.x >> 5);
+  if (F.f.skip_rec == nullptr || F.p.is_idr || mb >= n_mb) return;
+  SkipScratch& s = scr[threadIdx.x >> 5];
+  mb_ctx(s.ctx, F.p, F.f, mb % F.p.mb_w, mb / F.p.mb_w);
+  skip_prepass_mb(s.ctx, s, force_miss != 0);
 }
 
 struct Sched {
@@ -339,6 +350,12 @@
 }
 
 __device__ unsigned long long g_enc_stats[16];
+__device__ unsigned long long g_skip_stats[2];
+extern "C" int b2h264_debug_skip_stats(unsigned long long* out2, int reset) {
+  cudaError_t e = cudaMemcpyFromSymbol(out2, g_skip_stats, sizeof(g_skip_stats));
+  if (e == cudaSuccess && reset) { unsigned long long z[2] = {0, 0}; e = cudaMemcpyToSymbol(g_skip_stats, z, sizeof(z)); }
+  return (int)e;
+}
 #ifdef B2H264_PHASE_STATS
 namespace mbk { __device__ unsigned long long g_phase[32]; }
 extern "C" int b2h264_debug_phase_stats(unsigned long long* out32, int reset) {
@@ -385,6 +402,7 @@
     if ((stats & 1) && (threadIdx.x & 31) == 0) {
       atomicAdd(&g_enc_stats[2 * stage], (unsigned long long)(clock64() - t0));
       atomicAdd(&g_enc_stats[2 * stage + 1], 1ull);
+      if (stage == MBS_A && s.skip_hit) atomicAdd(&g_skip_stats[s.skip_hit - 1], 1ull);
     }
     return next;
   });
@@ -591,7 +609,7 @@
 }
 
 int enc_launch_frame(const StreamFrame* d_sf, const uint8_t* const* d_src, int n_streams, int w, int h, int mb_w, int mb_h,
-                     int* d_ws, void* d_stash, const void* tmap_ref, const void* d_tmap, int fast_mode, cudaStream_t st,
+                     int* d_ws, void* d_stash, const void* tmap_ref, const void* d_tmap, int fast_mode, int skip_prepass, cudaStream_t st,
                      cudaStream_t st_dbk, cudaEvent_t ev_ready, cudaEvent_t ev_dbk) {
   int rc;
   if (d_src) {
@@ -602,6 +620,11 @@
   if (fast_mode) {
     const int n_mb = mb_w * mb_h;
     k_vaa_sad8x8<<<dim3((n_mb + 7) / 8, n_streams), 256, 0, st>>>(d_sf, n_mb);
+    if ((rc = b2h264_launched())) return rc;
+  }
+  if (skip_prepass) {
+    const int n_mb = mb_w * mb_h;
+    k_skip_prepass<<<dim3((n_mb + SKIP_PP_WPC - 1) / SKIP_PP_WPC, n_streams), 32 * SKIP_PP_WPC, 0, st>>>(d_sf, n_mb, skip_prepass == 2);
     if ((rc = b2h264_launched())) return rc;
   }
   const int total = n_streams * mb_w * mb_h;
diff --git a/openh264_b200/csrc/enc_launch.h b/openh264_b200/csrc/enc_launch.h
--- a/openh264_b200/csrc/enc_launch.h
+++ b/openh264_b200/csrc/enc_launch.h
@@ -13,7 +13,9 @@
 int enc_launch_frame(const StreamFrame* d_sf, const uint8_t* const* d_src, int n_streams, int w, int h, int mb_w, int mb_h,
                      int* d_sched_ws, void* d_stash, const void* tmap_ref ,
                      const void* d_tmap ,
-                     int fast_mode , cudaStream_t st,
+                     int fast_mode ,
+                     int skip_prepass ,
+                     cudaStream_t st,
                      cudaStream_t st_dbk ,
                      cudaEvent_t ev_ready, cudaEvent_t ev_dbk );
 int enc_launch_deblock_expand(const StreamFrame* d_sf, int n_streams, int mb_w, int mb_h, int* d_sched_ws, cudaStream_t st,
diff --git a/openh264_b200/csrc/enc_mb.cuh b/openh264_b200/csrc/enc_mb.cuh
--- a/openh264_b200/csrc/enc_mb.cuh
+++ b/openh264_b200/csrc/enc_mb.cuh
@@ -62,6 +62,16 @@
   int16_t mvcand[5][2];
   int32_t win_x0, win_y0, win_ok;
   uint32_t t_last;
+  SkipRec skrec;
+  int32_t skip_hit;
+};
+
+struct alignas(16) SkipScratch {
+  uint8_t skip_pred[384];
+  uint8_t cur_y[256];
+  uint8_t cur_c[128];
+  int16_t coef[384];
+  MbCtx ctx;
 };
 static_assert(offsetof(MbScratch, skip_pred) == offsetof(MbScratch, pred_c) + 256 &&
               offsetof(MbScratch, qplane) == offsetof(MbScratch, skip_pred) + 384 && offsetof(MbScratch, coef) == offsetof(MbScratch, qplane) + 3 * 18 * 32 &&
@@ -122,7 +132,8 @@
   warp_sync();
 }
 
-MBK_HD void mb_load_cur(const MbCtx& c, MbScratch& s) {
+template <class Scratch>
+MBK_HD void mb_load_cur(const MbCtx& c, Scratch& s) {
   const uint8_t* y = c.f.cur[0] + (size_t)(c.mby * 16) * c.p.cur_stride_y + c.mbx * 16;
   for (int i = lane_id(); i < 64; i += MBK_WS) {
     const int r = i >> 2, c4 = (i & 3) << 2;
@@ -181,6 +192,8 @@
   if (l < 8 && (c.nb & nb_bit(l & 3)))
     hist = l < 4 ? ld_cg_u32(reinterpret_cast<const uint32_t*>(c.f.sad_cost + idx + nb_off(l & 3)))
                  : ld_cg_u32(reinterpret_cast<const uint32_t*>(&c.f.rec_info[idx + nb_off(l & 3)].skip_sad));
+  const bool skw_on = c.f.skip_rec != nullptr && l >= 8 && l < 12;
+  const uint32_t skw = skw_on ? reinterpret_cast<const uint32_t*>(c.f.skip_rec + idx)[l - 8] : 0u;
   const uint8_t* cy = c.f.cur[0] + (size_t)(c.mby * 16) * c.p.cur_stride_y + c.mbx * 16;
   const uint32_t cy0 = *reinterpret_cast<const uint32_t*>(cy + (size_t)(l >> 2) * c.p.cur_stride_y + ((l & 3) << 2));
   const uint32_t cy1 = *reinterpret_cast<const uint32_t*>(cy + (size_t)(8 + (l >> 2)) * c.p.cur_stride_y + ((l & 3) << 2));
@@ -215,6 +228,7 @@
   }
   if (l < 4) s.nb_sad[l] = (int32_t)hist;
   else if (l < 8) s.nb_skip_sad[l - 4] = (int32_t)hist;
+  if (skw_on) reinterpret_cast<uint32_t*>(&s.skrec)[l - 8] = skw;
   *reinterpret_cast<uint32_t*>(s.cur_y + (l >> 2) * 16 + ((l & 3) << 2)) = cy0;
   *reinterpret_cast<uint32_t*>(s.cur_y + (8 + (l >> 2)) * 16 + ((l & 3) << 2)) = cy1;
   *reinterpret_cast<uint32_t*>(s.cur_c + (l >> 4) * 64 + ((l >> 1) & 7) * 8 + ((l & 1) << 2)) = cc;
@@ -235,10 +249,26 @@
   mb_load_neighbors(c, s);
   mb_load_cur(c, s);
   mb_load_borders(c, s);
+  if (c.f.skip_rec != nullptr) s.skrec = c.f.skip_rec[idx];
 #endif
 }
 
-MBK_HD void mb_store_recon_skip(const MbCtx& c, MbScratch& s) {
+MBK_HD void mb_load_skip_pred(const MbCtx& c, MbScratch& s) {
+  const uint8_t* ry = c.f.rec[0] + (size_t)(c.mby * 16) * c.p.rec_stride_y + c.mbx * 16;
+  for (int i = lane_id(); i < 96; i += MBK_WS) {
+    uint32_t v;
+    if (i < 64) v = *reinterpret_cast<const uint32_t*>(ry + (size_t)(i >> 2) * c.p.rec_stride_y + ((i & 3) << 2));
+    else {
+      const int j = i - 64, pl = j >> 4, r = (j >> 1) & 7, c4 = (j & 1) << 2;
+      v = *reinterpret_cast<const uint32_t*>(c.f.rec[1 + pl] + (size_t)(c.mby * 8 + r) * c.p.rec_stride_c + c.mbx * 8 + c4);
+    }
+    *reinterpret_cast<uint32_t*>(s.skip_pred + 4 * i) = v;
+  }
+  warp_sync();
+}
+
+template <class Scratch>
+MBK_HD void mb_store_recon_skip(const MbCtx& c, Scratch& s) {
   uint8_t* ry = c.f.rec[0] + (size_t)(c.mby * 16) * c.p.rec_stride_y + c.mbx * 16;
   for (int i = lane_id(); i < 64; i += MBK_WS) {
     const int r = i >> 2, c4 = (i & 3) << 2;
diff --git a/openh264_b200/csrc/enc_types.h b/openh264_b200/csrc/enc_types.h
--- a/openh264_b200/csrc/enc_types.h
+++ b/openh264_b200/csrc/enc_types.h
@@ -30,6 +30,17 @@
   uint8_t mb_type;
   uint8_t pad[3];
 } RefMbInfo;
+
+typedef struct {
+  int16_t mv[2];
+  int32_t sad_mb;
+  int32_t cost_luma;
+  uint16_t sad_y;
+  uint8_t flags;
+  uint8_t pad;
+} SkipRec;
+#define SKIPREC_QUANT_OK 1
+#define SKIPREC_OUT_OF_RANGE 2
 
 typedef struct {
   uint8_t mb_type, cbp, qp, i16_mode;
@@ -102,4 +113,5 @@
   const DecMbAuxB* dec_aux_b;
   const uint8_t* prev_luma;
   int32_t* mb_bits;
+  SkipRec* skip_rec;
 } EncFramePtrs;
```

Result: slower. 4098, median of 6 (-10.9%).
